# wborgeaud/python-bulletproofs

Measured on AMD Instinct MI355X. Metric: Pippenger MSM scalar-point pairs/sec at n=2^20, higher is better.
Workload: dtype u32x9 (29-bit limbs, 256-bit modular integer); 1 GPU; MSM n=2^20 per GPU over secp256k1, uniform 256-bit scalars (SHA-256), points k_i*G, inputs resident in HBM, 64-byte result to host every step; pairs_per_gpu=1048576, pipeline=2 MSMs in flight (bpmi_msm_dev_enqueue / bpmi_msm_finish)

## Files before the change

### python-bulletproofs_amd/csrc/msm_host.hpp

```cpp
#pragma once

struct MsmGraphKey {
  int lane, slot, glv, small, opt_quad, opt_tail, opt_epl, opt_hist_threads, opt_hist_blocks;
  u32 w0, wcount;
  Segs segs;
  MsmGeom g;
  const void *ws, *pin;
};
struct MsmGraphEntry {
  MsmGraphKey key;
  hipGraph_t graph = nullptr;
  hipGraphExec_t exec = nullptr;
  u32 W = 0, nv = 0, c = 0; int tail = 2; TailOffs to;
};
struct MsmGraphCache { std::vector<MsmGraphEntry> entries; };
static void msm_graphs_clear(bpmi_ctx *ctx) {
  if (!ctx->graphs || ctx->graphs->entries.empty()) return;
  (void)sync_lanes(ctx);
  for (auto &e : ctx->graphs->entries) { if (e.exec) (void)hipGraphExecDestroy(e.exec); if (e.graph) (void)hipGraphDestroy(e.graph); }
  ctx->graphs->entries.clear();
}
static void msm_graph_key(MsmGraphKey &key, const bpmi_ctx *ctx, const MsmPlan &pl, int lane, int slot, const Segs &segs_in, u32 w0, u32 wcount) {
  memset(&key, 0, sizeof(key));
  key.lane = lane; key.slot = slot; key.glv = pl.glv; key.small = pl.small ? 1 : (pl.mid ? 2 : 0); key.opt_quad = ctx->opt_quad; key.opt_tail = ctx->opt_tail; key.opt_epl = ctx->opt_epl;
  key.opt_hist_threads = ctx->opt_hist_threads; key.opt_hist_blocks = ctx->opt_hist_blocks; key.w0 = w0; key.wcount = wcount;
  memcpy(&key.segs, &segs_in, sizeof(Segs)); memcpy(&key.g, &pl.g, sizeof(MsmGeom));
  key.ws = ctx->lane[lane].ws; key.pin = ctx->pend[slot].pin;
}
struct MsmCapture {
  bpmi_ctx *ctx; hipStream_t st; bpmi_ctx::PendingMsm &pd;
  MsmGraphKey key; bool open = false;
  MsmCapture(bpmi_ctx *c, hipStream_t s, bpmi_ctx::PendingMsm &p) : ctx(c), st(s), pd(p) {}
  ~MsmCapture() { if (open) { hipGraph_t g = nullptr; (void)hipStreamEndCapture(st, &g); if (g) (void)hipGraphDestroy(g); (void)hipGetLastError(); } }
  int begin(bool &replayed) {
    replayed = false;
    if (ctx->graphs)
      for (auto &e : ctx->graphs->entries)
        if (!memcmp(&e.key, &key, sizeof(key))) {
          HIPCHK(ctx, hipGraphLaunch(e.exec, st));
          replayed = true;
          return commit(e.W, e.nv, e.c, e.tail, e.to);
        }
    HIPCHK(ctx, hipStreamBeginCapture(st, hipStreamCaptureModeThreadLocal));
    open = true;
    return BPMI_OK;
  }
  int commit(u32 W_, u32 nv_, u32 c_, int tail_, const TailOffs &to_) {
    if (open) {
      MsmGraphEntry e;
      memcpy(&e.key, &key, sizeof(key)); e.W = W_; e.nv = nv_; e.c = c_; e.tail = tail_; e.to = to_;
      open = false;
      HIPCHK(ctx, hipStreamEndCapture(st, &e.graph));
      hipError_t ie = hipGraphInstantiate(&e.exec, e.graph, nullptr, nullptr, 0);
      if (ie != hipSuccess) { (void)hipGraphDestroy(e.graph); return fail(ctx, BPMI_E_HIP, std::string("hipGraphInstantiate: ") + hipGetErrorString(ie)); }
      if (!ctx->graphs) ctx->graphs = new MsmGraphCache();
      if (ctx->graphs->entries.size() >= 48) msm_graphs_clear(ctx);
      ctx->graphs->entries.push_back(e);
      HIPCHK(ctx, hipGraphLaunch(e.exec, st));
    }
    HIPCHK(ctx, hipEventRecord(pd.done, st));
    pd.active = true; pd.W = W_; pd.nv = nv_; pd.c = c_; pd.tail = tail_; pd.to = to_;
    HIPCHK(ctx, hipGetLastError());
    return BPMI_OK;
  }
};

static int msm_queue_mid(bpmi_ctx *ctx, hipStream_t st, const bpmi_ctx::PendingMsm &pd, const Segs &segs, const MsmGeom &g, const MsmWs &w, u32 *E_dst) {
  {
    StageTimer t(ctx, ST_ACCUM, st);
    MidPair mp;
    memset(&mp, 0, sizeof(mp));
    mp.segs[0] = segs; mp.g[0] = g; mp.E[0] = E_dst;
    hipLaunchKernelGGL(k_msm_mid, dim3(g.W, 1, g.nv), dim3(MID_THREADS), 0, st, mp);
  }
  debug_sync(ctx, "k_msm_mid", st);
  if (!ctx->opt_direct) HIPCHK(ctx, hipMemcpyAsync(pd.pin, w.E, 4ull * XYZZ_WORDS * g.W * g.nv, hipMemcpyDeviceToHost, st));
  return BPMI_OK;
}
static int msm_queue_small(bpmi_ctx *ctx, hipStream_t st, const bpmi_ctx::PendingMsm &pd, const Segs &segs, const MsmGeom &g, const MsmWs &w, u32 *E_dst) {
  const uint64_t n = segs.total;
  {
    StageTimer t(ctx, ST_ACCUM, st);
    const u32 threads = (u32)std::min<uint64_t>(256, (n + 63) / 64 * 64);
    const u32 S = (u32)std::min<uint64_t>(64, (n + 255) / 256);
    hipLaunchKernelGGL(k_msm_small, dim3(g.W, S), dim3(threads), 0, st, segs, g, S > 1 ? w.buckets : E_dst);
    if (S > 1) hipLaunchKernelGGL(k_small_combine, dim3(g.W), dim3(64), 0, st, w.buckets, S, E_dst);
  }
  debug_sync(ctx, "k_msm_small", st);
  if (!ctx->opt_direct) HIPCHK(ctx, hipMemcpyAsync(pd.pin, w.E, 4ull * XYZZ_WORDS * g.W, hipMemcpyDeviceToHost, st));
  return BPMI_OK;
}
static void msm_queue_sort_lds(bpmi_ctx *ctx, hipStream_t st, const Segs &segs, const MsmGeom &g, const MsmWs &w, const MsmRecode *rec = nullptr) {
  {
    StageTimer t(ctx, ST_DIGITS, st);
    const u32 ht = ctx->opt_hist_threads > 0 ? (u32)ctx->opt_hist_threads : 1024u;
    const u32 hb = (u32)std::min<uint64_t>(((uint64_t)(rec ? rec->real.n : g.n) + ht - 1) / ht, ctx->opt_hist_blocks > 0 ? (u32)ctx->opt_hist_blocks : 256u);
    CoarseScanOut so = {nullptr, nullptr, nullptr, nullptr};
    if (ctx->opt_histscan && !rec) { so.coarse_off = w.coarse_off; so.coarse_cursor = w.coarse_cursor; so.offG = w.off + g.G; so.ticket = w.coarse_hist + PART_MAX + 2; }
    if (rec) hipLaunchKernelGGL(k_fixed_recode, dim3(hb), dim3(ht), 0, st, rec->sc, rec->real, rec->n_scalars, rec->R, rec->Wv, g, w.P, w.coarse_hist, w.dig16, w.negs);
    else hipLaunchKernelGGL(k_coarse_hist, dim3(hb), dim3(ht), 0, st, segs, g, w.P, w.coarse_hist, w.dig16, w.negs, so);
  }
  debug_sync(ctx, "ST_DIGITS", st);
  if (!ctx->opt_histscan || rec) {
    StageTimer t(ctx, ST_SCAN, st);
    hipLaunchKernelGGL(k_coarse_scan, dim3(1), dim3(1024), 0, st, w.coarse_hist, w.P, w.coarse_off, w.coarse_cursor, w.off + g.G);
  }
  debug_sync(ctx, "ST_SCAN", st);
  {
    StageTimer t(ctx, ST_SCATTER, st);
    const u32 TS = g.n >= (1u << 19) ? PT_MAX : 4096u;
    hipLaunchKernelGGL(k_partition, dim3((g.n + TS - 1) / TS, g.W), dim3(PT_THREADS), 0, st, g, w.P, TS, w.coarse_off, w.coarse_cursor, w.dig16, w.negs, w.dig,
                       w.hist, w.coarse_hist + PART_MAX);
    const u32 nft = (u32)(((size_t)g.n * g.W + FINE_TILE - 1) / FINE_TILE);
    const u32 *any_heavy = w.coarse_hist + PART_MAX;
    if (!g.inblock) hipLaunchKernelGGL(k_fine_hist_heavy, dim3(nft), dim3(256), 0, st, g, w.P, w.coarse_off, w.dig, w.coarse_off + w.P, any_heavy, w.hist);
    hipLaunchKernelGGL(k_fine_sort_part, dim3(w.P), dim3(FINE_THREADS), 0, st, g, w.coarse_off, w.dig, w.hist, w.off, w.cursor, w.chunk_key, w.sidx, w.buckets);
    if (!g.inblock) hipLaunchKernelGGL(k_fine_scatter_heavy, dim3(nft), dim3(256), 0, st, g, w.P, w.coarse_off, w.dig, w.coarse_off + w.P, any_heavy, w.cursor, w.sidx);
    if (g.runs) {
      const u32 cap = msm_runs_cap(*ctx, g), nblk = msm_runs_blocks(g);
      const RunTable rt = {w.run_order, w.run_counts, w.run_flags, msm_runs_bins(cap), cap};
      hipLaunchKernelGGL(k_runs_hist, dim3(nblk), dim3(256), 0, st, g, w.off, rt);
      hipLaunchKernelGGL(k_runs_scatter, dim3(nblk), dim3(256), 0, st, g, w.off, rt);
    }
  }
  debug_sync(ctx, "ST_SCATTER", st);
}
static void msm_queue_sort_atomic(bpmi_ctx *ctx, hipStream_t st, const Segs &segs, const MsmGeom &g, const MsmWs &w) {
  const u32 nblk_n = (u32)std::min<uint64_t>(((uint64_t)g.n + 255) / 256, 8192);
  {
    StageTimer t(ctx, ST_DIGITS, st);
    hipLaunchKernelGGL(k_digits_hist, dim3(nblk_n), dim3(256), 0, st, segs, g, w.dig, w.hist);
  }
  debug_sync(ctx, "ST_DIGITS", st);
  {
    StageTimer t(ctx, ST_SCAN, st);
    hipLaunchKernelGGL(k_scan_partials, dim3(w.nscan_blocks), dim3(256), 0, st, w.hist, g.G, w.bsum);
    hipLaunchKernelGGL(k_scan_top, dim3(1), dim3(1024), 0, st, w.bsum, w.nscan_blocks, w.off, g.G);
    hipLaunchKernelGGL(k_scan_final, dim3(w.nscan_blocks), dim3(256), 0, st, w.hist, g.G, w.bsum, w.off, w.cursor);
  }
  debug_sync(ctx, "ST_SCAN", st);
  {
    StageTimer t(ctx, ST_SCATTER, st);
    hipLaunchKernelGGL(k_scatter, dim3(nblk_n), dim3(256), 0, st, g, w.dig, w.cursor, w.sidx);
    hipLaunchKernelGGL(k_chunk_keys, dim3((g.G + 255) / 256), dim3(256), 0, st, g, w.off, w.chunk_key);
  }
  debug_sync(ctx, "ST_SCATTER", st);
}
static int msm_queue_sort(bpmi_ctx *ctx, hipStream_t st, const Segs &segs, const MsmGeom &g, const MsmWs &w, const MsmRecode *rec = nullptr) {
  {
    StageTimer t(ctx, ST_MISC, st);
    if (w.P) HIPCHK(ctx, hipMemsetAsync(w.coarse_hist, 0, 4ull * COARSE_HIST_WORDS, st));
    else {
      HIPCHK(ctx, hipMemsetAsync(w.hist, 0, 4ull * g.G, st));
      HIPCHK(ctx, hipMemsetAsync(w.buckets, 0, 4ull * XYZZ_WORDS * g.G, st));
    }
  }
  debug_sync(ctx, "ST_MISC", st);
  if (w.P) msm_queue_sort_lds(ctx, st, segs, g, w, rec);
  else msm_queue_sort_atomic(ctx, st, segs, g, w);
  return BPMI_OK;
}
static int msm_queue_accumulate(bpmi_ctx *ctx, const MsmMode &mode, int lane, hipStream_t st, const Segs &segs, const MsmGeom &g, const MsmWs &w, bool glv) {
  const bool own_acc = mode.chained && ctx->opt_accum_stream && ctx->stream_acc;
  hipStream_t st_acc = own_acc ? ctx->stream_acc : st;
  Lane &l = ctx->lane[lane];
  if (own_acc) {
    HIPCHK(ctx, hipEventRecord(l.ev_sorted, st));
    HIPCHK(ctx, hipStreamWaitEvent(st_acc, l.ev_sorted, 0));
  } else if (mode.chained && !mode.free_run && ctx->accum_chain_lane >= 0 && ctx->accum_chain_lane != lane)
    HIPCHK(ctx, hipStreamWaitEvent(st, ctx->lane[ctx->accum_chain_lane].ev_accum, 0));
  {
    StageTimer t(ctx, ST_ACCUM, st_acc);
    auto kern = glv ? (g.fuse ? k_accum_l0<true, true> : k_accum_l0<true, false>) : (g.fuse ? k_accum_l0<false, true> : k_accum_l0<false, false>);
    const u32 *long_run = g.runs ? w.run_flags + RUN_FLAG_WORD : nullptr;
    if (g.runs) {
      auto runs = (!glv && segs_one_dense(segs)) ? k_accum_runs<true> : k_accum_runs<false>;
      hipLaunchKernelGGL(runs, dim3((g.G + 255) / 256), dim3(256), 0, st_acc, segs, g, w.off, w.sidx, w.run_order, w.run_flags, w.buckets);
    }
    hipLaunchKernelGGL(kern, dim3((w.nchunks + 255) / 256), dim3(256), 0, st_acc, segs, g, w.off, w.chunk_key, w.sidx, w.buckets, w.rec_key[0], w.rec_pt[0], long_run);
  }
  if (own_acc) {
    HIPCHK(ctx, hipEventRecord(l.ev_accum, st_acc));
    HIPCHK(ctx, hipStreamWaitEvent(st, l.ev_accum, 0));
  } else if (mode.chained) { HIPCHK(ctx, hipEventRecord(l.ev_accum, st)); ctx->accum_chain_lane = lane; }
  debug_sync(ctx, "ST_ACCUM", st);
  return BPMI_OK;
}
static void msm_queue_segscan(bpmi_ctx *ctx, hipStream_t st, const MsmGeom &g, const MsmWs &w) {
  {
    StageTimer t(ctx, ST_SEGSCAN, st);
    u32 R = w.rec0_max;
    int level = 1, src = 0;
    u32 *ticket = (w.P && ctx->opt_segfuse) ? w.coarse_hist + PART_MAX + 1 : nullptr;
    const u32 *long_run = g.runs ? w.run_flags + RUN_FLAG_WORD : nullptr;
    for (;;) {
      const u32 nb = (R + 255) / 256;
      if (nb > 128u || nb <= 1u) ticket = nullptr;
      hipLaunchKernelGGL(k_segscan, dim3(nb), dim3(256), 0, st, g, w.off, level, w.rec_key[src], w.rec_pt[src],
                         w.rec_key[src ^ 1], w.rec_pt[src ^ 1], w.buckets, ticket, long_run);
      if (g_debug_sync) { fprintf(stderr, "[bpmi] segscan level %d nb %u R %u\n", level, nb, R); debug_sync(ctx, "segscan level", st); }
      if (nb <= 1 || ticket) break;
      R = 2 * nb;
      src ^= 1;
      level++;
    }
  }
  debug_sync(ctx, "ST_SEGSCAN", st);
}
static TailOffs msm_queue_reduce(bpmi_ctx *ctx, hipStream_t st, const MsmGeom &g, const MsmWs &w, u32 *E_red) {
  const MsmReducePlan r = msm_reduce_plan(g, *ctx);
  {
    StageTimer t(ctx, ST_BREDUCE, st);
    if (g.B <= 256u) {
      if (ctx->opt_quad) hipLaunchKernelGGL(k_window_weighted_small_quad, dim3(g.W), dim3(g.B < 16u ? 64u : 4u * g.B), 0, st, g, w.buckets, E_red);
      else hipLaunchKernelGGL(k_window_weighted_small, dim3(g.W), dim3(g.B < 64u ? 64u : g.B), 0, st, g, w.buckets, E_red);
    } else {
      hipLaunchKernelGGL(k_digit_sums, dim3(r.grid1), dim3(256), 0, st, w.buckets, w.D, r.j1);
      if (ctx->opt_quad && ctx->opt_final_spread == 1 && w.P)
        hipLaunchKernelGGL(k_digit_final_spread<0>, dim3(g.W * 64u), dim3(64), 0, st, w.D, w.F, w.coarse_hist + PART_MAX + 8, E_red, r.j2, r.j2top, r.top_w);
      else if (ctx->opt_quad && ctx->opt_final_spread >= 2) {
        if (ctx->opt_final_spread == 2) hipLaunchKernelGGL(k_digit_final_spread<1>, dim3(g.W * 64u), dim3(64), 0, st, w.D, w.F, nullptr, E_red, r.j2, r.j2top, r.top_w);
        else hipLaunchKernelGGL(k_digit_final_spread<1>, dim3(g.W * 16u), dim3(256), 0, st, w.D, w.F, nullptr, E_red, r.j2, r.j2top, r.top_w);
        hipLaunchKernelGGL(k_digit_final_spread<2>, dim3(g.W * 4u), dim3(64), 0, st, w.D, w.F, nullptr, E_red, r.j2, r.j2top, r.top_w);
      }
      else if (ctx->opt_quad) hipLaunchKernelGGL(k_digit_final_quad, dim3(g.W * 4u), dim3(1024), 0, st, w.D, E_red, r.j2, r.j2top, r.top_w);
      else hipLaunchKernelGGL(k_digit_final, dim3(g.W * 4u), dim3(256), 0, st, w.D, E_red, r.j2, r.j2top, r.top_w);
    }
  }
  debug_sync(ctx, "ST_BREDUCE", st);
  return r.to;
}
static int msm_queue_tail(bpmi_ctx *ctx, hipStream_t st, const bpmi_ctx::PendingMsm &pd, const MsmGeom &g, const MsmWs &w, int tail, const TailOffs &to) {
  StageTimer t(ctx, ST_TAIL, st);
  if (tail == 1) {
    hipLaunchKernelGGL(k_tail, dim3(1), dim3(64), 0, st, w.E, g.W, g.c, to, ctx->opt_direct ? (u32 *)pd.pin : w.out);
    if (!ctx->opt_direct) HIPCHK(ctx, hipMemcpyAsync(pd.pin, w.out, 64, hipMemcpyDeviceToHost, st));
  } else if (!ctx->opt_direct)
    HIPCHK(ctx, hipMemcpyAsync(pd.pin, w.E, 4ull * XYZZ_WORDS * g.W * g.nv, hipMemcpyDeviceToHost, st));
  return BPMI_OK;
}

static int msm_enqueue(bpmi_ctx *ctx, const MsmMode &mode, int lane, int slot, const Segs &segs_in, u32 w0 = 0, u32 wcount = 0, int phase = 0,
                       const MsmRecode *rec = nullptr) {
  Segs segs = segs_in;
  const uint64_t n = segs.total;
  bpmi_ctx::PendingMsm &pd = ctx->pend[slot];
  if (pd.active) return fail(ctx, BPMI_E_STATE, "an MSM is still pending in this slot (bpmi_msm_finish it first)");
  if (n == 0) return BPMI_OK;
  if (n > BPMI_MAX_N) return fail(ctx, BPMI_E_ARG, "n exceeds BPMI_MAX_N");
  const MsmPlan pl = rec ? rec->plan : msm_pick_geometry(*ctx, mode, n, w0, wcount);
  MsmGeom g = pl.g;
  MsmWs w;
  msm_layout(g, w, nullptr, pl.glv);
  int rc = ensure_lane(ctx, lane);
  if (rc) return rc;
  rc = ensure_ws(ctx, w.total, lane);
  if (rc) return rc;
  msm_layout(g, w, (char *)ctx->lane[lane].ws, pl.glv);
  hipStream_t st = ctx->lane[lane].stream;
  rc = ensure_pin_slot(ctx, slot, std::max<size_t>(4096, 4ull * XYZZ_WORDS * g.W * 4));
  if (rc) return rc;
  const bool sort_ahead = !pl.mid && !pl.small && !pl.glv;
  if (phase == 1) {
    if (!sort_ahead) return BPMI_OK;
    if ((rc = msm_queue_sort(ctx, st, segs, g, w))) return rc;
    HIPCHK(ctx, hipGetLastError());
    return BPMI_OK;
  }
  MsmCapture cap(ctx, st, pd);
  if (phase == 0 && ctx->opt_graph && !ctx->prof && !g_debug_sync && !mode.chained && !rec) {
    msm_graph_key(cap.key, ctx, pl, lane, slot, segs_in, w0, wcount);
    bool replayed;
    rc = cap.begin(replayed);
    if (rc || replayed) return rc;
  }
  u32 *const E_dst = ctx->opt_direct ? (u32 *)pd.pin : w.E;
  if (pl.glv) {
    StageTimer t(ctx, ST_DIGITS, st);
    hipLaunchKernelGGL(k_glv_prepare, dim3((u32)((n + 255) / 256)), dim3(256), 0, st, segs, (u32)n, w.glv_sub, w.glv_neg, w.glv_bx);
    segs.glv_sub = w.glv_sub; segs.glv_neg = w.glv_neg; segs.glv_bx = w.glv_bx;
  }
  TailOffs to;
  memset(&to, 0, sizeof(to));
  to.nv = 1;
  int tail = 2;
  if (pl.mid) {
    g.nv = to.nv = mid_parts(*ctx, n);
    if ((rc = msm_queue_mid(ctx, st, pd, segs, g, w, E_dst))) return rc;
  } else if (pl.small) {
    if ((rc = msm_queue_small(ctx, st, pd, segs, g, w, E_dst))) return rc;
  } else {
    ctx->lane[lane].run_planned = g.runs; ctx->lane[lane].run_flags = w.P ? w.run_flags : nullptr;
    if (!(phase == 2 && sort_ahead) && (rc = msm_queue_sort(ctx, st, segs, g, w, rec))) return rc;
    if ((rc = msm_queue_accumulate(ctx, mode, lane, st, segs, g, w, pl.glv))) return rc;
    msm_queue_segscan(ctx, st, g, w);
    tail = wcount ? 2 : (ctx->opt_tail ? ctx->opt_tail : 2);
    to = msm_queue_reduce(ctx, st, g, w, tail == 1 ? w.E : E_dst);
    if ((rc = msm_queue_tail(ctx, st, pd, g, w, tail, to))) return rc;
  }
  return cap.commit(g.W, g.nv, g.c, tail, to);
}
static void msm_abandon_pending(bpmi_ctx *ctx, unsigned mine) {
  (void)sync_lanes(ctx);
  for (int s = 0; s < BPMI_LANES; s++) if ((mine >> s) & 1u) ctx->pend[s].active = false;
}
static int msm_finish(bpmi_ctx *ctx, int slot, uint8_t out[64]) {
  bpmi_ctx::PendingMsm &pd = ctx->pend[slot];
  if (!pd.active) { memset(out, 0, 64); return BPMI_OK; }
  pd.active = false;
  HIPCHK(ctx, wait_event(ctx, pd.done));
  const void *pin = pd.pin;
  if (pd.tail == 1) {
    memcpy(out, pin, 64);
  } else {
    bpmi_host::tail_combine(out, (const u32 *)pin, pd.W, pd.c, pd.to);
  }
  return BPMI_OK;
}
static int msm_run_split(bpmi_ctx *ctx, const Segs &segs, uint8_t out[64]) {
  const u32 c = pick_window_bits(*ctx, segs.total), W = 255u / c + 1u, Wa = W / 2;
  int rc = ensure_lane(ctx, 1);
  if (rc) return rc;
  HIPCHK(ctx, hipEventRecord(ctx->ev_fork, ctx->stream));
  HIPCHK(ctx, hipStreamWaitEvent(ctx->lane[1].stream, ctx->ev_fork, 0));
  rc = msm_enqueue(ctx, MsmMode{}, 0, 0, segs, 0, Wa);
  if (rc) return rc;
  rc = msm_enqueue(ctx, MsmMode{}, 1, 1, segs, Wa, W - Wa);
  if (rc) { msm_abandon_pending(ctx, 1u); return rc; }
  bpmi_ctx::PendingMsm &p0 = ctx->pend[0], &p1 = ctx->pend[1];
  HIPCHK(ctx, hipStreamSynchronize(ctx->stream));
  HIPCHK(ctx, hipStreamSynchronize(ctx->lane[1].stream));
  const size_t b0 = 4ull * XYZZ_WORDS * p0.W * p0.nv, b1 = 4ull * XYZZ_WORDS * p1.W * p1.nv;
  std::vector<u32> E((b0 + b1) / 4);
  memcpy(E.data(), p0.pin, b0);
  memcpy((char *)E.data() + b0, p1.pin, b1);
  bpmi_host::tail_combine(out, E.data(), W, c, p0.to);
  p0.active = p1.active = false;
  return BPMI_OK;
}
static int msm_finish_pair(bpmi_ctx *ctx, uint8_t out0[64], uint8_t out1[64]);
static int msm_run_sliced(bpmi_ctx *ctx, const Segs &segs, uint64_t K, uint8_t out[64]) {
  for (int s = 0; s < 2; s++) if (ctx->pend[s].active || ctx->pend[s].async) return fail(ctx, BPMI_E_STATE, "an MSM is still pending in this slot (bpmi_msm_finish it first)");
  int rc = ensure_lane(ctx, 1);
  if (rc) return rc;
  HIPCHK(ctx, hipEventRecord(ctx->ev_fork, ctx->stream));
  HIPCHK(ctx, hipStreamWaitEvent(ctx->lane[1].stream, ctx->ev_fork, 0));
  const uint64_t total = segs.total, per = (total + K - 1) / K;
  bpmi_host::pt acc;
  bpmi_host::pt_set_inf(acc);
  unsigned mine = 0;
  MsmMode mode;
  mode.chained = per >= (1u << 19);
  auto leave = [&](int code) { ctx->accum_chain_lane = -1; if (code) msm_abandon_pending(ctx, mine); return code; };
  auto take = [&](int slot) -> int {
    uint8_t part[64];
    mine &= ~(1u << slot);
    const int r = msm_finish(ctx, slot, part);
    if (r) return r;
    bpmi_host::pt p;
    bpmi_host::pt_from_affine(p, part);
    bpmi_host::pt_add(acc, acc, p);
    return BPMI_OK;
  };
  ctx->accum_chain_lane = -1;
  for (uint64_t k = 0; k < K; k++) {
    const int lane = (int)(k & 1);
    if (k >= 2) { rc = take(lane); if (rc) return leave(rc); }
    const MsmSlice sl = msm_slice(total, per, k);
    rc = msm_enqueue(ctx, mode, lane, lane, segs_slice(segs, sl.lo, sl.cnt));
    if (rc) return leave(rc);
    mine |= 1u << lane;
  }
  {
    uint8_t part[2][64];
    mine = 0;
    rc = msm_finish_pair(ctx, part[0], part[1]);
    if (rc) return leave(rc);
    for (uint64_t k = K - 2; k < K; k++) {
      bpmi_host::pt p;
      bpmi_host::pt_from_affine(p, part[k & 1]);
      bpmi_host::pt_add(acc, acc, p);
    }
  }
  bpmi_host::pt_to_affine(out, acc);
  return leave(BPMI_OK);
}
static int msm_run(bpmi_ctx *ctx, const Segs &segs, uint8_t out[64]) {
  if (segs.total > BPMI_MAX_N) return fail(ctx, BPMI_E_ARG, "n exceeds BPMI_MAX_N");
  {
    const uint64_t K = msm_slice_count(*ctx, segs);
    if (K > 1) return msm_run_sliced(ctx, segs, K, out);
  }
  if (ctx->opt_split == 1 && segs.total >= 2) return msm_run_split(ctx, segs, out);
  int rc = msm_enqueue(ctx, MsmMode{}, 0, 0, segs);
  if (rc) return rc;
  return msm_finish(ctx, 0, out);
}
static int msm_finish_pair(bpmi_ctx *ctx, uint8_t out0[64], uint8_t out1[64]) {
  if (!ctx->opt_tail_thread || !ctx->pend[0].active || !ctx->pend[1].active) {
    const int rc = msm_finish(ctx, 0, out0), rc1 = msm_finish(ctx, 1, out1);
    return rc ? rc : rc1;
  }
  if (!ctx->helper) ctx->helper = new HostHelper();
  bpmi_ctx::PendingMsm &pd = ctx->pend[1];
  hipError_t e1 = hipSuccess;
  const int dev = ctx->device;
  ctx->helper->submit([&pd, &e1, out1, dev, ctx] {
    (void)hipSetDevice(dev);
    e1 = wait_event(ctx, pd.done);
    if (e1 != hipSuccess) return;
    if (pd.tail == 1) memcpy(out1, pd.pin, 64);
    else bpmi_host::tail_combine(out1, (const u32 *)pd.pin, pd.W, pd.c, pd.to);
  });
  const int rc = msm_finish(ctx, 0, out0);
  ctx->helper->wait();
  pd.active = false;
  if (rc) return rc;
  HIPCHK(ctx, e1);
  return BPMI_OK;
}
static int msm_enqueue_small_pair(bpmi_ctx *ctx, const Segs &s0, const Segs &s1, bool mid) {
  bpmi_ctx::PendingMsm &p0 = ctx->pend[0], &p1 = ctx->pend[1];
  if (p0.active || p1.active) return fail(ctx, BPMI_E_STATE, "an MSM is still pending in this slot (bpmi_msm_finish it first)");
  SmallPair sp;
  CombinePair cp;
  MidPair mp;
  memset(&mp, 0, sizeof(mp));
  const Segs *ss[2] = {&s0, &s1};
  size_t off[2], total = 0;
  MsmWs w[2];
  MsmGeom gg[2];
  const u32 c = mid ? MID_C : SMALL_C;
  for (int j = 0; j < 2; j++) {
    MsmGeom &g = gg[j];
    memset(&g, 0, sizeof(g));
    g.n = ss[j]->total; g.c = c; g.W = 255u / g.c + 1u; g.w0 = 0; g.B = 1u << (g.c - 1); g.G = g.W * g.B; g.L = 8; g.nv = 1;
    msm_layout(g, w[j], nullptr);
    off[j] = total;
    total += align_up(w[j].total, 256);
  }
  int rc = ensure_ws(ctx, total);
  if (rc) return rc;
  const u32 parts = mid ? mid_parts(*ctx, std::max(s0.total, s1.total)) : 1u;
  const size_t eb = 4ull * XYZZ_WORDS * gg[0].W * parts;
  for (int j = 0; j < 2; j++) { rc = ensure_pin_slot(ctx, j, eb); if (rc) return rc; }
  u32 Smax = 1, threads = 64;
  for (int j = 0; j < 2; j++) {
    msm_layout(gg[j], w[j], (char *)ctx->lane[0].ws + off[j]);
    const uint64_t n = ss[j]->total;
    const u32 S = (u32)std::min<uint64_t>(64, (n + 255) / 256);
    u32 *const E_dst = ctx->opt_direct ? (u32 *)ctx->pend[j].pin : w[j].E;
    sp.segs[j] = *ss[j]; sp.g[j] = gg[j]; sp.S[j] = S; sp.out[j] = S > 1 ? w[j].buckets : E_dst;
    cp.part[j] = w[j].buckets; cp.S[j] = S; cp.E[j] = E_dst;
    mp.segs[j] = *ss[j]; mp.g[j] = gg[j]; mp.E[j] = E_dst;
    Smax = std::max(Smax, S);
    threads = std::max(threads, (u32)std::min<uint64_t>(256, (n + 63) / 64 * 64));
  }
  hipStream_t st = ctx->stream;
  {
    StageTimer t(ctx, ST_ACCUM, st);
    if (mid) hipLaunchKernelGGL(k_msm_mid, dim3(gg[0].W, 2, parts), dim3(MID_THREADS), 0, st, mp);
    else {
      hipLaunchKernelGGL(k_msm_small_pair, dim3(gg[0].W, Smax, 2), dim3(threads), 0, st, sp);
      if (Smax > 1) hipLaunchKernelGGL(k_small_combine_pair, dim3(gg[0].W, 2), dim3(64), 0, st, cp);
    }
  }
  debug_sync(ctx, "k_msm_small_pair / k_msm_mid", st);
  TailOffs to;
  memset(&to, 0, sizeof(to));
  to.nv = parts;
  unsigned mine = 0;
  auto queue_results = [&]() -> int {
    for (int j = 0; j < 2; j++) {
      bpmi_ctx::PendingMsm &pd = ctx->pend[j];
      if (!ctx->opt_direct) HIPCHK(ctx, hipMemcpyAsync(pd.pin, w[j].E, eb, hipMemcpyDeviceToHost, st));
      HIPCHK(ctx, hipEventRecord(pd.done, st));
      pd.active = true; pd.W = gg[j].W; pd.nv = parts; pd.c = c; pd.tail = 2; pd.to = to;
      mine |= 1u << j;
    }
    HIPCHK(ctx, hipGetLastError());
    return BPMI_OK;
  };
  rc = queue_results();
  if (rc && mine) msm_abandon_pending(ctx, mine);
  return rc;
}
static int msm_run_pair(bpmi_ctx *ctx, const Segs &s0, uint8_t out0[64], const Segs &s1, uint8_t out1[64]) {
  if (s0.total > BPMI_MAX_N || s1.total > BPMI_MAX_N) return fail(ctx, BPMI_E_ARG, "n exceeds BPMI_MAX_N");
  {
    const uint64_t small_max = ctx->opt_small < 0 ? 0 : (ctx->opt_small ? (uint64_t)ctx->opt_small : SMALL_N_DEFAULT);
    const uint64_t mid_min = ctx->opt_mid_min > 0 ? (uint64_t)ctx->opt_mid_min : MID_MIN_DEFAULT;
    const uint64_t big = std::max<uint64_t>(s0.total, s1.total);
    const bool mid = ctx->opt_mid_min >= 0 && big >= mid_min && big <= MID_NMAX && ctx->opt_glv <= 0;
    if (ctx->opt_pair1 && ctx->opt_c == 0 && s0.total && s1.total && (mid || big <= small_max)) {
      int rc = msm_enqueue_small_pair(ctx, s0, s1, mid);
      if (rc) return rc;
      return msm_finish_pair(ctx, out0, out1);
    }
  }
  int rc = ensure_lane(ctx, 1);
  if (rc) return rc;
  HIPCHK(ctx, hipEventRecord(ctx->ev_fork, ctx->stream));
  HIPCHK(ctx, hipStreamWaitEvent(ctx->lane[1].stream, ctx->ev_fork, 0));
  const bool big = s0.total >= (1u << 19) && s1.total >= (1u << 19);
  const bool sched = ctx->opt_pair_sched && big && !ctx->opt_graph;
  const bool chain = sched || (ctx->opt_pair_chain && big);
  MsmMode mode;
  mode.chained = chain;
  mode.beside = ctx->opt_pair_rounds != 1 && big;
  if (chain) ctx->accum_chain_lane = -1;
  auto leave = [&](int code) { if (chain) ctx->accum_chain_lane = -1; return code; };
  const bool phases = sched || (ctx->opt_pair_phases && !chain && !ctx->opt_graph && s0.total >= (1u << 15) && s1.total >= (1u << 15));
  if (phases) {
    rc = msm_enqueue(ctx, mode, 0, 0, s0, 0, 0, 1);
    if (rc == BPMI_OK) rc = msm_enqueue(ctx, mode, 1, 1, s1, 0, 0, 1);
    if (rc) { msm_abandon_pending(ctx, 0u); return leave(rc); }
    if (sched) {
      hipError_t e = hipEventRecord(ctx->ev_join, ctx->lane[1].stream);
      if (e == hipSuccess) e = hipStreamWaitEvent(ctx->stream, ctx->ev_join, 0);
      if (e != hipSuccess) { msm_abandon_pending(ctx, 0u); return leave(fail(ctx, BPMI_E_HIP, std::string("msm_run_pair: ") + hipGetErrorString(e))); }
    }
  }
  rc = msm_enqueue(ctx, mode, 0, 0, s0, 0, 0, phases ? 2 : 0);
  if (rc == BPMI_OK) {
    rc = msm_enqueue(ctx, mode, 1, 1, s1, 0, 0, phases ? 2 : 0);
    if (rc) msm_abandon_pending(ctx, 1u);
  }
  leave(0);
  if (rc) return rc;
  return msm_finish_pair(ctx, out0, out1);
}
```

### python-bulletproofs_amd/csrc/msm_kernels.hpp

```cpp
#pragma once

__device__ __forceinline__ void raise_priority(u32 on) { if (on) __builtin_amdgcn_s_setprio(3); }
__device__ __forceinline__ u32 geom_wide(const MsmGeom &g, u32 w) { return (g.top2 && w + g.top2 >= g.W) ? 1u : 0u; }
__device__ __forceinline__ u32 geom_slot(const MsmGeom &g, u32 w) { return (g.top2 && w + g.top2 > g.W) ? 2u * w + g.top2 - g.W : w; }

__device__ __forceinline__ bool load_digit_source(sc &s, const Segs &segs, u32 i) {
  if (segs.glv_sub) {
    const uint4 t = *reinterpret_cast<const uint4 *>(segs.glv_sub + 4ull * i);
    s.v[0] = t.x; s.v[1] = t.y; s.v[2] = t.z; s.v[3] = t.w;
    s.v[4] = s.v[5] = s.v[6] = s.v[7] = 0;
    return segs.glv_neg[i] != 0;
  }
  load_words8(s.v, seg_scalar(segs, i));
  sc_reduce_once(s);
  const bool neg = sc_is_high(s);
  if (neg) sc_neg(s, s);
  return neg;
}
template <typename F>
__device__ __forceinline__ bool for_each_digit_raw(const Segs &segs, const MsmGeom &g, u32 i, F f) {
  sc s;
  const bool neg = load_digit_source(s, segs, i);
  u32 carry = 0;
  const u32 wend = g.w0 + g.W;
  for (u32 w = 0; w < wend; w++) {
    const u32 wd = g.c + geom_wide(g, w);
    const u32 t = (s.v[0] & ((1u << wd) - 1u)) + carry;
#pragma unroll
    for (int k = 0; k < 7; k++) s.v[k] = (u32)((((u64)s.v[k + 1] << 32) | s.v[k]) >> wd);
    s.v[7] >>= wd;
    u32 b, sign;
    if (t > (1u << (wd - 1u))) { b = (1u << wd) - t; sign = 1; carry = 1; }
    else { b = t; sign = 0; carry = 0; }
    if (w >= g.w0) f(w - g.w0, b, b ? sign : 0u);
  }
  return neg;
}
template <typename F>
__device__ __forceinline__ void for_each_digit(const Segs &segs, const MsmGeom &g, u32 i, F f) {
  sc s;
  const bool neg = load_digit_source(s, segs, i);
  u32 carry = 0;
  const u32 wend = g.w0 + g.W;
  for (u32 w = 0; w < wend; w++) {
    const u32 wd = g.c + geom_wide(g, w);
    const u32 t = (s.v[0] & ((1u << wd) - 1u)) + carry;
#pragma unroll
    for (int k = 0; k < 7; k++) s.v[k] = (u32)((((u64)s.v[k + 1] << 32) | s.v[k]) >> wd);
    s.v[7] >>= wd;
    u32 b, sign;
    if (t > (1u << (wd - 1u))) { b = (1u << wd) - t; sign = 1; carry = 1; }
    else { b = t; sign = 0; carry = 0; }
    if (w >= g.w0) f(w - g.w0, b, b ? (sign ^ (u32)neg) : 0u);
  }
}

__global__ void __launch_bounds__(256) k_glv_prepare(Segs segs, u32 n, u32 *__restrict__ sub, unsigned char *__restrict__ neg, u32 *__restrict__ bx) {
  const u32 i = blockIdx.x * blockDim.x + threadIdx.x;
  if (i >= n) return;
  sc k;
  load_words8(k.v, seg_scalar(segs, i));
  sc_reduce_once(k);
  u32 k1[4], k2[4];
  bool n1, n2;
  glv_split(k1, n1, k2, n2, k);
  uint4 *o = reinterpret_cast<uint4 *>(sub + 8ull * i);
  o[0] = make_uint4(k1[0], k1[1], k1[2], k1[3]);
  o[1] = make_uint4(k2[0], k2[1], k2[2], k2[3]);
  neg[2ull * i] = n1 ? 1 : 0;
  neg[2ull * i + 1] = n2 ? 1 : 0;
  u32 w[8];
  load_words8(w, seg_point(segs, i));
  fe x, r, c;
  fe_from_words(x, w);
  fe_mul_beta(r, x);
  fe_canon(c, r);
  fe_to_words(w, c);
  store_words8(bx + 8ull * i, w);
}

__global__ void __launch_bounds__(256) k_digits_hist(Segs segs, MsmGeom g, u32 *__restrict__ dig, u32 *__restrict__ hist) {
  raise_priority(g.prio & PRIO_SORT);
  const u32 stride = gridDim.x * blockDim.x;
  for (u32 i = blockIdx.x * blockDim.x + threadIdx.x; i < g.n; i += stride) {
    for_each_digit(segs, g, i, [&](u32 w, u32 b, u32 sign) {
      dig[(u64)w * g.n + i] = b | (sign << 31);
      const u32 key = b ? (w * g.B + b - 1u) : 0xFFFFFFFFu;
      const unsigned long long act = __ballot(1);
      const u32 first = __builtin_amdgcn_readfirstlane(key);
      const unsigned long long same = __ballot(key == first);
      if (same == act) {
        if (first != 0xFFFFFFFFu) {
          const u32 lane_rank = __builtin_amdgcn_mbcnt_hi((u32)(act >> 32), __builtin_amdgcn_mbcnt_lo((u32)act, 0));
          if (lane_rank == 0) atomicAdd(&hist[first], (u32)__popcll(act));
        }
      } else if (b) {
        atomicAdd(&hist[key], 1u);
      }
    });
  }
}

#define FINE_CAP 12288
#define DIG_NONE 0xFFFFu
struct CoarseScanOut { u32 *coarse_off, *coarse_cursor, *offG, *ticket; };
__global__ void __launch_bounds__(1024) k_coarse_hist(Segs segs, MsmGeom g, u32 P, u32 *coarse_hist, unsigned short *__restrict__ dig16,
                                                     unsigned char *__restrict__ negs, CoarseScanOut scan) {
  raise_priority(g.prio & PRIO_SORT);
  __shared__ u32 lh[PART_MAX];
  __shared__ u32 s_last;
  for (u32 p = threadIdx.x; p < P; p += blockDim.x) lh[p] = 0;
  __syncthreads();
  const u32 Bc = g.B >> 8;
  const u32 stride = gridDim.x * blockDim.x;
  for (u32 i = blockIdx.x * blockDim.x + threadIdx.x; i < g.n; i += stride) {
    const bool neg = for_each_digit_raw(segs, g, i, [&](u32 w, u32 b, u32 dsign) {
      dig16[(u64)w * g.n + i] = (unsigned short)(b ? ((b - 1u) | (dsign << 15)) : DIG_NONE);
      if (b) atomicAdd(&lh[geom_slot(g, w) * Bc + ((b - 1u) >> 8)], 1u);
    });
    negs[i] = neg ? 1 : 0;
  }
  __syncthreads();
  for (u32 p = threadIdx.x; p < P; p += blockDim.x) { const u32 v = lh[p]; if (v) atomicAdd(&coarse_hist[p], v); }
  if (!scan.ticket) return;
  __threadfence();
  __syncthreads();
  if (threadIdx.x == 0) s_last = (atomicAdd(scan.ticket, 1u) == gridDim.x - 1u) ? 1u : 0u;
  __syncthreads();
  if (!s_last) return;
  __threadfence();
  const u32 tid = threadIdx.x, nt = blockDim.x, per = (P + nt - 1u) / nt;
  u32 loc[8], sum = 0;
#pragma unroll
  for (u32 k = 0; k < 8u; k++) {
    const u32 idx = tid * per + k;
    loc[k] = (k < per && idx < P) ? __atomic_load_n(&coarse_hist[idx], __ATOMIC_RELAXED) : 0u;
    sum += loc[k];
  }
  lh[tid] = sum;
  __syncthreads();
  for (u32 d = 1; d < nt; d <<= 1) {
    const u32 v = tid >= d ? lh[tid - d] : 0u;
    __syncthreads();
    lh[tid] += v;
    __syncthreads();
  }
  u32 excl = lh[tid] - sum;
#pragma unroll
  for (u32 k = 0; k < 8u; k++) {
    const u32 idx = tid * per + k;
    if (k < per && idx < P) { scan.coarse_off[idx] = excl; scan.coarse_cursor[idx] = excl; excl += loc[k]; }
  }
  if (tid == nt - 1u) { scan.coarse_off[P] = lh[tid]; *scan.offG = lh[tid]; }
}
__global__ void __launch_bounds__(1024) k_coarse_scan(const u32 *__restrict__ coarse_hist, u32 P, u32 *__restrict__ coarse_off,
                                                      u32 *__restrict__ coarse_cursor, u32 *__restrict__ offG) {
  __shared__ u32 sh[1024];
  const u32 tid = threadIdx.x;
  const u32 a = (2u * tid < P) ? coarse_hist[2u * tid] : 0u, b = (2u * tid + 1u < P) ? coarse_hist[2u * tid + 1u] : 0u;
  sh[tid] = a + b;
  __syncthreads();
  for (u32 d = 1; d < 1024u; d <<= 1) {
    const u32 v = tid >= d ? sh[tid - d] : 0u;
    __syncthreads();
    sh[tid] += v;
    __syncthreads();
  }
  const u32 excl = sh[tid] - (a + b);
  if (2u * tid < P) { coarse_off[2u * tid] = excl; coarse_cursor[2u * tid] = excl; }
  if (2u * tid + 1u < P) { coarse_off[2u * tid + 1u] = excl + a; coarse_cursor[2u * tid + 1u] = excl + a; }
  if (tid == 1023u) { coarse_off[P] = sh[1023]; *offG = sh[1023]; }
}
#define PT_MAX 16384
#define PT_THREADS 1024u
struct alignas(8) PartSigns { unsigned char b[8]; };
__global__ void __launch_bounds__(PT_THREADS) k_partition(MsmGeom g, u32 P, u32 TS, const u32 *__restrict__ coarse_off, u32 *__restrict__ coarse_cursor,
                                                          const unsigned short *__restrict__ dig16, const unsigned char *__restrict__ negs,
                                                          u32 *__restrict__ part, u32 *__restrict__ fine_hist, u32 *__restrict__ any_heavy) {
  constexpr u32 THREADS = PT_THREADS;
  static_assert((PT_MAX / 8u) % THREADS == 0u, "k_partition: whole vectors per thread");
  constexpr u32 NV = PT_MAX / 8u / THREADS;
  raise_priority(g.prio & PRIO_SORT);
  __shared__ u32 cnt[128], excl[128], delta[128];
  __shared__ u32 s_out[PT_MAX];
  const u32 w = blockIdx.y, tid = threadIdx.x;
  const u32 Bc0 = g.B >> 8, Bc = Bc0 << geom_wide(g, w), pbase = geom_slot(g, w) * Bc0;
  const u32 lin = blockIdx.y * gridDim.x + blockIdx.x, nblk = gridDim.x * gridDim.y;
  if (!g.inblock) for (u32 p = lin; p < P; p += nblk) {
    if (coarse_off[p + 1] - coarse_off[p] > FINE_CAP) {
      if (tid < 256u) fine_hist[p * 256u + tid] = 0;
      if (tid == 0) *any_heavy = 1u;
    }
  }
  const u32 i0 = blockIdx.x * TS;
  const u32 i1 = (i0 + TS < g.n) ? i0 + TS : g.n;
  const u64 wn = (u64)w * g.n;
  const unsigned short *dw = dig16 + wn;
  const u32 span = i1 - i0, mis = (u32)((0u - (u32)((wn + i0) & 7ull)) & 7u);
  const u32 head = mis < span ? mis : span;
  const u32 a0 = i0 + head, nvec = (i1 - a0) >> 3, t0 = a0 + 8u * nvec;
  const u32 nscal = head + (i1 - t0);
  const u32 is = tid < head ? i0 + tid : t0 + (tid - head);
  uint4 cv[NV];
  PartSigns sv[NV];
  u32 cs = DIG_NONE, ss = 0;
#pragma unroll
  for (u32 k = 0; k < NV; k++) {
    const u32 v = k * THREADS + tid;
    cv[k] = make_uint4(0xFFFFFFFFu, 0xFFFFFFFFu, 0xFFFFFFFFu, 0xFFFFFFFFu);
    if (v < nvec) {
      cv[k] = *reinterpret_cast<const uint4 *>(dw + a0 + 8u * v);
      __builtin_memcpy(&sv[k], negs + a0 + 8u * v, 8);
    }
  }
  if (tid < nscal) { cs = dw[is]; ss = negs[is]; }
  if (tid < 128u) cnt[tid] = 0;
  __syncthreads();
#pragma unroll
  for (u32 k = 0; k < NV; k++) {
    const u32 q[4] = {cv[k].x, cv[k].y, cv[k].z, cv[k].w};
#pragma unroll
    for (u32 e = 0; e < 8u; e++) {
      const u32 code = (q[e >> 1] >> (16u * (e & 1u))) & 0xFFFFu;
      if (code != DIG_NONE) atomicAdd(&cnt[(code & 0x7FFFu) >> 8], 1u);
    }
  }
  if (cs != DIG_NONE) atomicAdd(&cnt[(cs & 0x7FFFu) >> 8], 1u);
  __syncthreads();
  u32 c = 0;
  if (tid < 128u) { c = tid < Bc ? cnt[tid] : 0u; excl[tid] = c; }
  __syncthreads();
  for (u32 d = 1; d < 128u; d <<= 1) {
    u32 v = 0;
    if (tid < 128u && tid >= d) v = excl[tid - d];
    __syncthreads();
    if (tid < 128u) excl[tid] += v;
    __syncthreads();
  }
  if (tid < 128u) {
    const u32 start = excl[tid] - c;
    excl[tid] = start;
    cnt[tid] = start;
    if (c) delta[tid] = atomicAdd(&coarse_cursor[pbase + tid], c) - start;
  }
  __syncthreads();
#pragma unroll
  for (u32 k = 0; k < NV; k++) {
    const u32 q[4] = {cv[k].x, cv[k].y, cv[k].z, cv[k].w};
    const u32 ib = a0 + 8u * (k * THREADS + tid);
#pragma unroll
    for (u32 e = 0; e < 8u; e++) {
      const u32 code = (q[e >> 1] >> (16u * (e & 1u))) & 0xFFFFu;
      if (code != DIG_NONE) {
        const u32 kk = code & 0x7FFFu;
        s_out[atomicAdd(&cnt[kk >> 8], 1u)] = ((kk & 255u) << 24) | (((code >> 15) ^ (u32)sv[k].b[e]) << 23) | (ib + e);
      }
    }
  }
  if (cs != DIG_NONE) {
    const u32 kk = cs & 0x7FFFu;
    s_out[atomicAdd(&cnt[kk >> 8], 1u)] = ((kk & 255u) << 24) | (((cs >> 15) ^ ss) << 23) | is;
  }
  __syncthreads();
  const u32 wave = tid >> 6, lane = tid & 63u, nwaves = THREADS >> 6;
  for (u32 p = wave; p < Bc; p += nwaves) {
    const u32 lo = excl[p], hi = cnt[p], dl = delta[p];
    for (u32 j = lo + lane; j < hi; j += 64u) part[dl + j] = s_out[j];
  }
}
#define CHUNK_FILL_OWN 16u
__device__ __forceinline__ void fill_chunk_keys(u32 *__restrict__ chunk_key, u32 L, u32 key, u32 lo, u32 hi) {
  const u32 t0 = (lo + L - 1u) / L;
  const u32 t1 = hi > lo ? (u32)(((u64)hi + L - 1u) / L) : t0;
  const bool big = t1 - t0 > CHUNK_FILL_OWN;
  if (!big) for (u32 t = t0; t < t1; t++) chunk_key[t] = key;
  unsigned long long m = __ballot(big);
  const u32 lane = __builtin_amdgcn_mbcnt_hi(~0u, __builtin_amdgcn_mbcnt_lo(~0u, 0u));
  while (m) {
    const int src = __ffsll((long long)m) - 1;
    m &= m - 1ull;
    const u32 k = (u32)__shfl((int)key, src, 64), a = (u32)__shfl((int)t0, src, 64), b = (u32)__shfl((int)t1, src, 64);
    for (u32 t = a + lane; t < b; t += 64u) chunk_key[t] = k;
  }
}
#define FINE_THREADS 512
__device__ __forceinline__ u32 lds_take_slot(u32 *bins, u32 bin) {
  const u32 lane = __builtin_amdgcn_mbcnt_hi(~0u, __builtin_amdgcn_mbcnt_lo(~0u, 0u));
  u32 pos = 0;
  bool done = false;
  for (int it = 0; it < 4; it++) {
    const unsigned long long rem = __ballot(!done);
    if (rem == 0ull) break;
    const u32 first = (u32)__shfl((int)bin, __ffsll((long long)rem) - 1, 64);
    const bool match = !done && bin == first;
    const unsigned long long m = __ballot(match);
    if (match) {
      const u32 rank = (u32)__popcll(m & ((1ull << lane) - 1ull));
      u32 basepos = 0;
      if (rank == 0) basepos = atomicAdd(&bins[first], (u32)__popcll(m));
      basepos = (u32)__shfl((int)basepos, __ffsll((long long)m) - 1, 64);
      pos = basepos + rank;
      done = true;
    }
  }
  if (!done) pos = atomicAdd(&bins[bin], 1u);
  return pos;
}
__global__ void __launch_bounds__(FINE_THREADS) k_fine_sort_part(MsmGeom g, const u32 *__restrict__ coarse_off, const u32 *__restrict__ part,
                                                                  const u32 *__restrict__ fine_hist, u32 *__restrict__ off, u32 *__restrict__ cursor,
                                                                  u32 *__restrict__ chunk_key, u32 *__restrict__ sidx, u32 *__restrict__ buckets) {
  raise_priority(g.prio & PRIO_SORT);
  __shared__ u32 bins[256];
  __shared__ u32 s_out[FINE_CAP];
  const u32 p = blockIdx.x, tid = threadIdx.x;
  const u32 base = coarse_off[p], m = coarse_off[p + 1] - base;
  const bool big = m > FINE_CAP;
  const bool heavy = big && !g.inblock;
  if (tid < 256u) bins[tid] = heavy ? fine_hist[p * 256u + tid] : 0u;
  __syncthreads();
  if (!heavy) {
    if (big) for (u32 i = tid; i < m; i += FINE_THREADS) (void)lds_take_slot(bins, part[base + i] >> 24);
    else for (u32 i = tid; i < m; i += FINE_THREADS) atomicAdd(&bins[part[base + i] >> 24], 1u);
    __syncthreads();
  }
  u32 cnt = 0;
  if (tid < 256u) cnt = bins[tid];
  for (u32 d = 1; d < 256u; d <<= 1) {
    u32 v = 0;
    if (tid < 256u && tid >= d) v = bins[tid - d];
    __syncthreads();
    if (tid < 256u) bins[tid] += v;
    __syncthreads();
  }
  if (tid < 256u) {
    const u32 start = bins[tid] - cnt;
    const u32 key = p * 256u + tid;
    off[key] = base + start;
    fill_chunk_keys(chunk_key, g.L, key, base + start, base + start + cnt);
    if (heavy) cursor[key] = base + start;
    if (cnt == 0) {
      xyzz inf;
      xyzz_set_inf(inf);
      xyzz_store_g(buckets + (u64)key * XYZZ_WORDS, inf);
    }
  }
  if (heavy) return;
  __syncthreads();
  if (tid < 256u) bins[tid] -= cnt;
  __syncthreads();
  if (big) {
    for (u32 i = tid; i < m; i += FINE_THREADS) {
      const u32 e = part[base + i];
      sidx[base + lds_take_slot(bins, e >> 24)] = (e & 0x7FFFFFu) | ((e & 0x800000u) << 8);
    }
    return;
  }
  for (u32 i = tid; i < m; i += FINE_THREADS) {
    const u32 e = part[base + i];
    s_out[atomicAdd(&bins[e >> 24], 1u)] = (e & 0x7FFFFFu) | ((e & 0x800000u) << 8);
  }
  __syncthreads();
  for (u32 i = tid; i < m; i += FINE_THREADS) sidx[base + i] = s_out[i];
}
#define FINE_BINS 4096
struct FineTile {
  u32 j0, j1;
  u32 p_first;
};
__device__ __forceinline__ FineTile fine_tile_setup(const u32 *__restrict__ coarse_off, u32 P, u32 E, u32 *s_off) {
  for (u32 i = threadIdx.x; i <= P; i += 256u) s_off[i] = coarse_off[i];
  __syncthreads();
  FineTile t;
  t.j0 = blockIdx.x * FINE_TILE;
  t.j1 = (t.j0 + FINE_TILE < E) ? t.j0 + FINE_TILE : E;
  u32 lo = 0, hi = P;
  while (hi - lo > 1) { const u32 mid = (lo + hi) >> 1; if (s_off[mid] <= t.j0) lo = mid; else hi = mid; }
  t.p_first = lo;
  return t;
}
__device__ __forceinline__ u32 fine_partition_of(const u32 *s_off, u32 P, u32 pcur, u32 j) {
  u32 lo = pcur + 1u, hi = P - 1u;
  while (lo < hi) { const u32 mid = (lo + hi) >> 1; if (s_off[mid + 1] > j) hi = mid; else lo = mid + 1u; }
  return lo;
}
__global__ void __launch_bounds__(256) k_fine_hist_heavy(MsmGeom g, u32 P, const u32 *__restrict__ coarse_off, const u32 *__restrict__ part,
                                                         const u32 *__restrict__ offE, const u32 *__restrict__ any_heavy, u32 *__restrict__ fine_hist) {
  raise_priority(g.prio & PRIO_SORT);
  __shared__ u32 s_off[PART_MAX + 1];
  __shared__ u32 bins[FINE_BINS];
  if (!*any_heavy) return;
  const u32 E = offE[0];
  if (blockIdx.x * FINE_TILE >= E) return;
  const FineTile t = fine_tile_setup(coarse_off, P, E, s_off);
  for (u32 i = threadIdx.x; i < FINE_BINS; i += 256u) bins[i] = 0;
  __syncthreads();
  const u32 g_first = t.p_first * 256u;
  u32 pcur = t.p_first, bound = s_off[pcur + 1];
  bool heavy = bound - s_off[pcur] > FINE_CAP;
  for (u32 j = t.j0 + threadIdx.x; j < t.j1; j += 256u) {
    if (j >= bound) { pcur = fine_partition_of(s_off, P, pcur, j); bound = s_off[pcur + 1]; heavy = bound - s_off[pcur] > FINE_CAP; }
    if (heavy) {
      const u32 key = pcur * 256u + (part[j] >> 24);
      const u32 rel = key - g_first;
      if (rel < FINE_BINS) atomicAdd(&bins[rel], 1u); else atomicAdd(&fine_hist[key], 1u);
    }
  }
  __syncthreads();
  for (u32 i = threadIdx.x; i < FINE_BINS; i += 256u) { const u32 v = bins[i]; if (v) atomicAdd(&fine_hist[g_first + i], v); }
}
__global__ void __launch_bounds__(256) k_fine_scatter_heavy(MsmGeom g, u32 P, const u32 *__restrict__ coarse_off, const u32 *__restrict__ part,
                                                            const u32 *__restrict__ offE, const u32 *__restrict__ any_heavy, u32 *__restrict__ cursor,
                                                            u32 *__restrict__ sidx) {
  raise_priority(g.prio & PRIO_SORT);
  __shared__ u32 s_off[PART_MAX + 1];
  __shared__ u32 bins[FINE_BINS];
  if (!*any_heavy) return;
  const u32 E = offE[0];
  if (blockIdx.x * FINE_TILE >= E) return;
  const FineTile t = fine_tile_setup(coarse_off, P, E, s_off);
  for (u32 i = threadIdx.x; i < FINE_BINS; i += 256u) bins[i] = 0;
  __syncthreads();
  const u32 g_first = t.p_first * 256u;
  u32 pcur = t.p_first, bound = s_off[pcur + 1];
  bool heavy = bound - s_off[pcur] > FINE_CAP;
  for (u32 j = t.j0 + threadIdx.x; j < t.j1; j += 256u) {
    if (j >= bound) { pcur = fine_partition_of(s_off, P, pcur, j); bound = s_off[pcur + 1]; heavy = bound - s_off[pcur] > FINE_CAP; }
    if (heavy) {
      const u32 rel = pcur * 256u + (part[j] >> 24) - g_first;
      if (rel < FINE_BINS) atomicAdd(&bins[rel], 1u);
    }
  }
  __syncthreads();
  for (u32 i = threadIdx.x; i < FINE_BINS; i += 256u) { const u32 v = bins[i]; if (v) bins[i] = atomicAdd(&cursor[g_first + i], v); }
  __syncthreads();
  pcur = t.p_first; bound = s_off[pcur + 1];
  heavy = bound - s_off[pcur] > FINE_CAP;
  for (u32 j = t.j0 + threadIdx.x; j < t.j1; j += 256u) {
    if (j >= bound) { pcur = fine_partition_of(s_off, P, pcur, j); bound = s_off[pcur + 1]; heavy = bound - s_off[pcur] > FINE_CAP; }
    if (heavy) {
      const u32 e = part[j];
      const u32 key = pcur * 256u + (e >> 24);
      const u32 rel = key - g_first;
      const u32 pos = (rel < FINE_BINS) ? atomicAdd(&bins[rel], 1u) : atomicAdd(&cursor[key], 1u);
      sidx[pos] = (e & 0x7FFFFFu) | ((e & 0x800000u) << 8);
    }
  }
}
__global__ void __launch_bounds__(256) k_chunk_keys(MsmGeom g, const u32 *__restrict__ off, u32 *__restrict__ chunk_key) {
  raise_priority(g.prio & PRIO_SORT);
  const u32 key = blockIdx.x * blockDim.x + threadIdx.x;
  const bool valid = key < g.G;
  const u32 lo = valid ? off[key] : 0u, hi = valid ? off[key + 1] : 0u;
  fill_chunk_keys(chunk_key, g.L, key, lo, hi);
}

__global__ void __launch_bounds__(256) k_scan_partials(const u32 *__restrict__ hist, u32 G, u32 *__restrict__ bsum) {
  __shared__ u32 red[256];
  const u32 base = blockIdx.x * SCAN_TILE + threadIdx.x * SCAN_PER_THREAD;
  u32 s = 0;
#pragma unroll
  for (int k = 0; k < SCAN_PER_THREAD; k++) { const u32 j = base + k; if (j < G) s += hist[j]; }
  red[threadIdx.x] = s;
  __syncthreads();
  for (int d = 128; d > 0; d >>= 1) { if (threadIdx.x < d) red[threadIdx.x] += red[threadIdx.x + d]; __syncthreads(); }
  if (threadIdx.x == 0) bsum[blockIdx.x] = red[0];
}
__global__ void __launch_bounds__(1024) k_scan_top(u32 *__restrict__ bsum, u32 nb, u32 *__restrict__ off, u32 G) {
  __shared__ u32 sh[1024];
  u32 running = 0;
  for (u32 base = 0; base < nb; base += 1024) {
    const u32 j = base + threadIdx.x;
    const u32 v = j < nb ? bsum[j] : 0;
    sh[threadIdx.x] = v;
    __syncthreads();
    for (int d = 1; d < 1024; d <<= 1) {
      u32 t = threadIdx.x >= d ? sh[threadIdx.x - d] : 0;
      __syncthreads();
      sh[threadIdx.x] += t;
      __syncthreads();
    }
    if (j < nb) bsum[j] = running + sh[threadIdx.x] - v;
    const u32 tot = sh[1023];
    __syncthreads();
    running += tot;
  }
  if (threadIdx.x == 0) off[G] = running;
}
__global__ void __launch_bounds__(256) k_scan_final(const u32 *__restrict__ hist, u32 G, const u32 *__restrict__ bsum,
                                                    u32 *__restrict__ off, u32 *__restrict__ cursor) {
  __shared__ u32 sh[256];
  const u32 base = blockIdx.x * SCAN_TILE + threadIdx.x * SCAN_PER_THREAD;
  u32 v[SCAN_PER_THREAD];
  u32 s = 0;
#pragma unroll
  for (int k = 0; k < SCAN_PER_THREAD; k++) { const u32 j = base + k; v[k] = j < G ? hist[j] : 0; s += v[k]; }
  sh[threadIdx.x] = s;
  __syncthreads();
  for (int d = 1; d < 256; d <<= 1) {
    u32 t = threadIdx.x >= d ? sh[threadIdx.x - d] : 0;
    __syncthreads();
    sh[threadIdx.x] += t;
    __syncthreads();
  }
  u32 run = bsum[blockIdx.x] + sh[threadIdx.x] - s;
#pragma unroll
  for (int k = 0; k < SCAN_PER_THREAD; k++) {
    const u32 j = base + k;
    if (j < G) { off[j] = run; cursor[j] = run; }
    run += v[k];
  }
}

__global__ void __launch_bounds__(256) k_scatter(MsmGeom g, const u32 *__restrict__ dig, u32 *__restrict__ cursor,
                                                 u32 *__restrict__ sidx) {
  raise_priority(g.prio & PRIO_SORT);
  const u32 stride = gridDim.x * blockDim.x;
  for (u32 w = 0; w < g.W; w++) {
    for (u32 i = blockIdx.x * blockDim.x + threadIdx.x; i < g.n; i += stride) {
      const u32 d = dig[(u64)w * g.n + i];
      const u32 b = d & 0x7FFFFFFFu;
      const u32 key = b ? (w * g.B + b - 1u) : 0xFFFFFFFFu;
      const unsigned long long act = __ballot(1);
      const u32 first = __builtin_amdgcn_readfirstlane(key);
      const unsigned long long same = __ballot(key == first);
      u32 pos = 0;
      if (same == act) {
        if (first != 0xFFFFFFFFu) {
          const u32 lane_rank = __builtin_amdgcn_mbcnt_hi((u32)(act >> 32), __builtin_amdgcn_mbcnt_lo((u32)act, 0));
          u32 basepos = 0;
          if (lane_rank == 0) basepos = atomicAdd(&cursor[first], (u32)__popcll(act));
          basepos = __builtin_amdgcn_readfirstlane(basepos);
          pos = basepos + lane_rank;
        }
      } else if (b) {
        pos = atomicAdd(&cursor[key], 1u);
      }
      if (b) sidx[pos] = i | (d & 0x80000000u);
    }
  }
}

__device__ __forceinline__ void xyzz_shfl_up(xyzz &r, const xyzz &a, int d) {
#pragma unroll
  for (int i = 0; i < 9; i++) {
    r.X.v[i] = (u32)__shfl_up((int)a.X.v[i], d, 64);
    r.Y.v[i] = (u32)__shfl_up((int)a.Y.v[i], d, 64);
    r.ZZ.v[i] = (u32)__shfl_up((int)a.ZZ.v[i], d, 64);
    r.ZZZ.v[i] = (u32)__shfl_up((int)a.ZZZ.v[i], d, 64);
  }
}
template <bool GLV, bool FUSE> __global__ void __launch_bounds__(256) k_accum_l0(Segs segs, MsmGeom g, const u32 *__restrict__ off,
                                                  const u32 *__restrict__ chunk_key, const u32 *__restrict__ sidx,
                                                  u32 *__restrict__ buckets, u32 *__restrict__ rec_key, u32 *__restrict__ rec_pt,
                                                  const u32 *__restrict__ long_run) {
  __shared__ u32 s_head[FUSE ? 256 * LDS_STRIDE : 1];
  if (long_run && !*long_run) return;
  const u32 E = off[g.G];
  const u64 t = (u64)blockIdx.x * blockDim.x + threadIdx.x;
  const u64 start = t * g.L;
  const bool valid = start < E;
  if (!FUSE) { if (!valid) return; }
  else if (__ballot(valid) == 0ull) return;
  const u32 end = (u32)((start + g.L < E) ? start + g.L : E);
  xyzz acc;
  xyzz_set_inf(acc);
  u32 cur = valid ? chunk_key[t] : 0u;
  const u32 hk = cur;
  bool first = true;
  if (valid) {
  u32 boundary = off[cur + 1];
  u32 boundary2 = off[cur + 2 < g.G ? cur + 2 : g.G];
  u32 e_next = sidx[start];
  u32 e_next2 = (start + 1 < end) ? sidx[start + 1] : 0u;
  u32 w_next[16];
  load_entry_point<GLV>(w_next, segs, e_next & 0x7FFFFFFFu);
  for (u32 j = (u32)start; j < end; j++) {
    const u32 e = e_next;
    affine P;
    affine_from_words(P, w_next);
    asm volatile("" : "+v"(P.x.v[0]), "+v"(P.x.v[1]), "+v"(P.x.v[2]), "+v"(P.x.v[3]), "+v"(P.x.v[4]), "+v"(P.x.v[5]), "+v"(P.x.v[6]),
                 "+v"(P.x.v[7]), "+v"(P.x.v[8]), "+v"(P.y.v[0]), "+v"(P.y.v[1]), "+v"(P.y.v[2]), "+v"(P.y.v[3]), "+v"(P.y.v[4]),
                 "+v"(P.y.v[5]), "+v"(P.y.v[6]), "+v"(P.y.v[7]), "+v"(P.y.v[8]));
    if (j + 1 < end) {
      e_next = e_next2;
      if (j + 2 < end) e_next2 = sidx[j + 2];
      load_entry_point<GLV>(w_next, segs, e_next & 0x7FFFFFFFu);
    }
    if (j == boundary) {
      if (first) {
        if (FUSE) xyzz_store(s_head + threadIdx.x * LDS_STRIDE, acc);
        else { rec_key[2 * t] = cur; xyzz_store_g(rec_pt + (2 * t) * XYZZ_WORDS, acc); }
        first = false;
      }
      else xyzz_store_g(buckets + (u64)cur * XYZZ_WORDS, acc);
      xyzz_set_inf(acc);
      cur++; boundary = boundary2;
      if (boundary == j) {
        u32 steps = 0;
        do { cur++; boundary = off[cur + 1]; steps++; } while (boundary == j && steps < 8u);
        if (boundary == j) {
          u32 lo = cur + 1u, hi = g.G - 1u;
          while (lo < hi) { const u32 mid = (lo + hi) >> 1; if (off[mid + 1] > j) hi = mid; else lo = mid + 1u; }
          cur = lo; boundary = off[cur + 1];
        }
      }
      boundary2 = off[cur + 2 < g.G ? cur + 2 : g.G];
    }
    xyzz_madd_signed(acc, P, (e >> 31) != 0);
  }
  }
  if (!FUSE) {
    if (first) {
      rec_key[2 * t] = cur; xyzz_store_g(rec_pt + (2 * t) * XYZZ_WORDS, acc);
      xyzz_set_inf(acc);
    }
    rec_key[2 * t + 1] = cur;
    xyzz_store_g(rec_pt + (2 * t + 1) * XYZZ_WORDS, acc);
    return;
  }
  const u32 lane = threadIdx.x & 63u;
  const u32 gw = (u32)(t >> 6);
  const bool single = first;
  const u32 tk = cur;
  const u32 prev_tk = (u32)__shfl_up((int)tk, 1, 64);
  const bool link = valid && lane > 0u && prev_tk == hk;
  bool F = !(valid && single && link);
  for (u32 d = 1; d < 64u; d <<= 1) {
    const bool take = !F;
    if (__ballot(take) == 0ull) break;
    xyzz o;
    xyzz_shfl_up(o, acc, (int)d);
    const bool oF = __shfl_up((int)F, (int)d, 64) != 0;
    if (take) { xyzz_add(acc, o, acc); F = oF; }
  }
  const u32 first_key = (u32)__shfl((int)hk, 0, 64);
  const bool next_valid = __shfl_down((int)valid, 1, 64) != 0, next_link = __shfl_down((int)link, 1, 64) != 0;
  const bool last = valid && (lane == 63u || !next_valid);
  xyzz Sp;
  xyzz_shfl_up(Sp, acc, 1);
  const bool s_done = valid && (last || !next_link);
  const bool s_is_head = tk == first_key;
  {
    u32 *dst = s_is_head ? rec_pt + (u64)(2u * gw) * XYZZ_WORDS : (last ? rec_pt + (u64)(2u * gw + 1u) * XYZZ_WORDS : buckets + (u64)tk * XYZZ_WORDS);
    if (s_done) xyzz_store_g(dst, acc);
  }
  if (last) {
    rec_key[2u * gw + 1u] = tk;
    if (s_is_head) {
      xyzz_set_inf(acc);
      xyzz_store_g(rec_pt + (u64)(2u * gw + 1u) * XYZZ_WORDS, acc);
    }
  }
  const bool has_head = valid && !single;
  if (__ballot(has_head) != 0ull) {
    if (has_head) xyzz_load(acc, s_head + threadIdx.x * LDS_STRIDE); else xyzz_set_inf(acc);
    if (__ballot(has_head && link) != 0ull) { if (has_head && link) xyzz_add(acc, Sp, acc); }
    u32 *dst = (hk == first_key) ? rec_pt + (u64)(2u * gw) * XYZZ_WORDS : buckets + (u64)hk * XYZZ_WORDS;
    if (has_head) xyzz_store_g(dst, acc);
  }
  if (lane == 0u) rec_key[2u * gw] = first_key;
}

__device__ __forceinline__ u32 records_at_level(u32 E, u32 L, u32 fuse, int level, bool &is_final) {
  is_final = false;
  if (E == 0) return 0;
  const u32 chunks = (E + L - 1) / L;
  u32 R = 2u * (fuse ? (chunks + 63u) / 64u : chunks);
  for (int l = 1; l < level; l++) {
    const u32 nb = (R + 255u) / 256u;
    if (nb <= 1) return 0;
    R = 2u * nb;
  }
  is_final = ((R + 255u) / 256u) <= 1;
  return R;
}

__global__ void __launch_bounds__(256) k_segscan(MsmGeom g, const u32 *__restrict__ off, int level,
                                                 const u32 *in_key, const u32 *in_pt,
                                                 u32 *out_key, u32 *out_pt, u32 *__restrict__ buckets, u32 *ticket, const u32 *__restrict__ long_run) {
  if (long_run && !*long_run) return;
  raise_priority(g.prio & PRIO_SCAN);
  __shared__ u32 s_key[256];
  __shared__ u32 s_val[256 * LDS_STRIDE];
  __shared__ u32 s_last;
  bool is_final;
  u32 R = records_at_level(off[g.G], g.L, g.fuse, level, is_final);
  u32 nb = (R + 255u) / 256u;
  if (blockIdx.x >= nb) return;
  const u32 tid = threadIdx.x;
  u32 blk = blockIdx.x;
  for (;;) {
    const u32 j = blk * 256u + tid;
    const bool valid = j < R;
    const u32 key = valid ? in_key[j] : 0xFFFFFFFFu;
    xyzz val;
    if (valid) xyzz_load_g(val, in_pt + (u64)j * XYZZ_WORDS); else xyzz_set_inf(val);
    s_key[tid] = key;
    __syncthreads();
    for (u32 d = 1; d < 256; d <<= 1) {
      const bool act = valid && tid >= d && s_key[tid - d] == key;
      if (!__syncthreads_or(act)) break;
      xyzz_store(s_val + tid * LDS_STRIDE, val);
      __syncthreads();
      if (act) {
        xyzz other;
        xyzz_load(other, s_val + (tid - d) * LDS_STRIDE);
        xyzz_add(val, other, val);
      }
      __syncthreads();
    }
    const u32 last_idx = (R - blk * 256u >= 256u) ? 255u : (R - blk * 256u - 1u);
    const bool run_end = valid && ((tid == last_idx) || (s_key[tid + (tid < 255u ? 1u : 0u)] != key));
    if (run_end) {
      const u32 first_key = s_key[0], last_key = s_key[last_idx];
      const bool to_bucket = is_final || (key != first_key && key != last_key);
      const bool is_head = !to_bucket && (key == first_key);
      const u32 slot = 2u * blk + (is_head ? 0u : 1u);
      u32 *dst = to_bucket ? buckets + (u64)key * XYZZ_WORDS : out_pt + (u64)slot * XYZZ_WORDS;
      if (!to_bucket) out_key[slot] = key;
      xyzz_store_g(dst, val);
      if (is_head && first_key == last_key) {
        xyzz inf;
        xyzz_set_inf(inf);
        out_key[slot + 1u] = key;
        xyzz_store_g(out_pt + (u64)(slot + 1u) * XYZZ_WORDS, inf);
      }
    }
    if (is_final || !ticket || nb > 128u) return;
    __threadfence();
    __syncthreads();
    if (tid == 0) s_last = (atomicAdd(ticket, 1u) == nb - 1u) ? 1u : 0u;
    __syncthreads();
    if (!s_last) return;
    __threadfence();
    R = 2u * nb; nb = 1; blk = 0; is_final = true;
    in_key = out_key; in_pt = out_pt;
  }
}

struct RunTable { u32 *order, *counts, *flags; u32 nbins, cap; };
template <u32 N> __device__ __forceinline__ void run_lengths(u32 (&len)[N], const u32 *__restrict__ off, u32 k0, u32 stride, u32 k1) {
#pragma unroll
  for (u32 k = 0; k < N; k++) { const u32 key = k0 + k * stride; len[k] = key < k1 ? off[key + 1] - off[key] : 0u; }
}
__global__ void __launch_bounds__(256) k_runs_hist(MsmGeom g, const u32 *__restrict__ off, RunTable rt) {
  raise_priority(g.prio & PRIO_SORT);
  __shared__ u32 bins[RUN_BINS];
  for (u32 i = threadIdx.x; i < rt.nbins; i += 256u) bins[i] = 0;
  __syncthreads();
  const u32 k0 = blockIdx.x * RUN_SLICE, k1 = (k0 + RUN_SLICE < g.G) ? k0 + RUN_SLICE : g.G;
  u32 len[RUN_SLICE / 256u];
  run_lengths(len, off, k0 + threadIdx.x, 256u, k1);
  bool longer = false;
#pragma unroll
  for (u32 k = 0; k < RUN_SLICE / 256u; k++) {
    if (len[k]) atomicAdd(&bins[len[k] < rt.nbins ? len[k] : rt.nbins - 1u], 1u);
    longer |= len[k] > rt.cap;
  }
  __syncthreads();
  for (u32 i = threadIdx.x; i < rt.nbins; i += 256u) rt.counts[(rt.nbins - 1u - i) * gridDim.x + blockIdx.x] = bins[i];
  if (longer) rt.flags[RUN_FLAG_WORD] = 1u;
}
__global__ void __launch_bounds__(256) k_runs_scatter(MsmGeom g, const u32 *__restrict__ off, RunTable rt) {
  raise_priority(g.prio & PRIO_SORT);
  __shared__ u32 s_base[RUN_BINS];
  __shared__ u32 s_wave[4][RUN_BINS];
  __shared__ u32 s_scan[256];
  if (rt.flags[RUN_FLAG_WORD]) return;
  const u32 tid = threadIdx.x, nblk = gridDim.x;
  const u32 wave = tid >> 6, lane = tid & 63u;
  const u32 k0 = blockIdx.x * RUN_SLICE + wave * (RUN_SLICE / 4u);
  const u32 k1 = (k0 + RUN_SLICE / 4u < g.G) ? k0 + RUN_SLICE / 4u : g.G;
  u32 len[RUN_SLICE / 256u];
  run_lengths(len, off, k0 + lane, 64u, k1);
  const u32 M = rt.nbins * nblk, per = ((M + 255u) / 256u + 3u) & ~3u;
  const u32 i0 = tid * per < M ? tid * per : M, i1 = i0 + per < M ? i0 + per : M;
  u32 sum = 0;
  {
    u32 i = i0;
#pragma unroll 4
    for (; i + 4u <= i1; i += 4u) { const uint4 v = *reinterpret_cast<const uint4 *>(rt.counts + i); sum += v.x + v.y + v.z + v.w; }
    for (; i < i1; i++) sum += rt.counts[i];
  }
  s_scan[tid] = sum;
  for (u32 i = tid; i < 4u * RUN_BINS; i += 256u) (&s_wave[0][0])[i] = 0;
  __syncthreads();
  for (u32 d = 1; d < 256u; d <<= 1) {
    const u32 v = tid >= d ? s_scan[tid - d] : 0u;
    __syncthreads();
    s_scan[tid] += v;
    __syncthreads();
  }
  {
    u32 run = s_scan[tid] - sum, row = i0 / nblk, blk = i0 % nblk;
    for (u32 i = i0; i < i1; i++) {
      if (blk == blockIdx.x) s_base[rt.nbins - 1u - row] = run;
      run += rt.counts[i];
      if (++blk == nblk) { blk = 0; row++; }
    }
  }
  if (blockIdx.x == 0 && tid == 255u) rt.flags[RUN_COUNT_WORD] = s_scan[255];
#pragma unroll
  for (u32 k = 0; k < RUN_SLICE / 256u; k++)
    if (len[k]) atomicAdd(&s_wave[wave][len[k] < rt.nbins ? len[k] : rt.nbins - 1u], 1u);
  __syncthreads();
  for (u32 cls = tid; cls < rt.nbins; cls += 256u) {
    u32 b = s_base[cls];
    for (u32 w = 0; w < 4u; w++) { const u32 c = s_wave[w][cls]; s_wave[w][cls] = b; b += c; }
  }
  __syncthreads();
#pragma unroll
  for (u32 k = 0; k < RUN_SLICE / 256u; k++)
    if (len[k]) rt.order[atomicAdd(&s_wave[wave][len[k] < rt.nbins ? len[k] : rt.nbins - 1u], 1u)] = k0 + lane + k * 64u;
}
template <bool DENSE> __device__ __forceinline__ void runs_load_point(u32 w[16], const Segs &segs, u32 idx) {
  if (DENSE) load_words16(w, segs.pts[0] + 16ull * idx);
  else load_entry_point<false>(w, segs, idx);
}
template <bool DENSE> __device__ __forceinline__ void runs_next_entry(affine &P, u32 &e, u32 (&w_next)[16], u32 &e_next, u32 &e_next2, const Segs &segs,
                                                                      const u32 *__restrict__ sidx, u32 j, u32 end) {
  e = e_next;
  affine_from_words(P, w_next);
  asm volatile("" : "+v"(P.x.v[0]), "+v"(P.x.v[1]), "+v"(P.x.v[2]), "+v"(P.x.v[3]), "+v"(P.x.v[4]), "+v"(P.x.v[5]), "+v"(P.x.v[6]),
               "+v"(P.x.v[7]), "+v"(P.x.v[8]), "+v"(P.y.v[0]), "+v"(P.y.v[1]), "+v"(P.y.v[2]), "+v"(P.y.v[3]), "+v"(P.y.v[4]),
               "+v"(P.y.v[5]), "+v"(P.y.v[6]), "+v"(P.y.v[7]), "+v"(P.y.v[8]));
  if (j + 1 < end) {
    e_next = e_next2;
    if (j + 2 < end) e_next2 = sidx[j + 2];
    runs_load_point<DENSE>(w_next, segs, e_next & 0x7FFFFFFFu);
  }
}
__device__ __forceinline__ void runs_signed_y(fe &sy, const fe &y, bool negate) {
  fe_neg(sy, y);
#pragma unroll
  for (int k = 0; k < 9; k++) sy.v[k] = negate ? sy.v[k] : y.v[k];
}
template <bool DENSE> __global__ void __launch_bounds__(256) k_accum_runs(Segs segs, MsmGeom g, const u32 *__restrict__ off, const u32 *__restrict__ sidx,
                                                    const u32 *__restrict__ order, const u32 *__restrict__ flags, u32 *__restrict__ buckets) {
  if (flags[RUN_FLAG_WORD]) return;
  const u32 t = blockIdx.x * blockDim.x + threadIdx.x;
  if (t >= flags[RUN_COUNT_WORD]) return;
  const u32 b = order[t];
  const u32 start = off[b], end = off[b + 1];
  xyzz acc;
  u32 e_next = sidx[start];
  u32 e_next2 = (start + 1 < end) ? sidx[start + 1] : 0u;
  u32 w_next[16];
  runs_load_point<DENSE>(w_next, segs, e_next & 0x7FFFFFFFu);
  u32 j = start, e;
  affine P;
  fe sy;
  runs_next_entry<DENSE>(P, e, w_next, e_next, e_next2, segs, sidx, j, end);
  bool fin = !affine_is_inf(P);
  runs_signed_y(sy, P.y, (e >> 31) != 0);
  if (fin) { acc.X = P.x; fe_carry(acc.Y, sy); fe_set_one(acc.ZZ); fe_set_one(acc.ZZZ); }
  else xyzz_set_inf(acc);
  j++;
  if (j < end) {
    runs_next_entry<DENSE>(P, e, w_next, e_next, e_next2, segs, sidx, j, end);
    if (!affine_is_inf(P)) {
      runs_signed_y(sy, P.y, (e >> 31) != 0);
      if (fin) xyzz_mmadd(acc, acc.X, acc.Y, P.x, sy);
      else { acc.X = P.x; fe_carry(acc.Y, sy); fe_set_one(acc.ZZ); fe_set_one(acc.ZZZ); }
    }
    j++;
  }
  for (; j < end; j++) {
    runs_next_entry<DENSE>(P, e, w_next, e_next, e_next2, segs, sidx, j, end);
    xyzz_madd_signed(acc, P, (e >> 31) != 0);
  }
  xyzz_store_g(buckets + (u64)b * XYZZ_WORDS, acc);
}

__device__ __forceinline__ void block_tree_sum(xyzz &val, u32 *s_val) {
  const u32 tid = threadIdx.x;
  for (u32 d = blockDim.x >> 1; d > 0; d >>= 1) {
    xyzz_store(s_val + tid * LDS_STRIDE, val);
    __syncthreads();
    if (tid < d) {
      xyzz other;
      xyzz_load(other, s_val + (tid + d) * LDS_STRIDE);
      xyzz_add(val, val, other);
    }
    __syncthreads();
  }
}


__device__ __forceinline__ void xyzz_shfl_xor(xyzz &r, const xyzz &a, int mask) {
#pragma unroll
  for (int i = 0; i < 9; i++) {
    r.X.v[i] = (u32)__shfl_xor((int)a.X.v[i], mask, 64);
    r.Y.v[i] = (u32)__shfl_xor((int)a.Y.v[i], mask, 64);
    r.ZZ.v[i] = (u32)__shfl_xor((int)a.ZZ.v[i], mask, 64);
    r.ZZZ.v[i] = (u32)__shfl_xor((int)a.ZZZ.v[i], mask, 64);
  }
}
__device__ __forceinline__ void xyzz_shfl_down(xyzz &r, const xyzz &a, int d) {
#pragma unroll
  for (int i = 0; i < 9; i++) {
    r.X.v[i] = (u32)__shfl_down((int)a.X.v[i], d, 64);
    r.Y.v[i] = (u32)__shfl_down((int)a.Y.v[i], d, 64);
    r.ZZ.v[i] = (u32)__shfl_down((int)a.ZZ.v[i], d, 64);
    r.ZZZ.v[i] = (u32)__shfl_down((int)a.ZZZ.v[i], d, 64);
  }
}
__device__ __forceinline__ void xyzz_shfl_down16(xyzz &r, const xyzz &a, int d) {
#pragma unroll
  for (int i = 0; i < 9; i++) {
    r.X.v[i] = (u32)__shfl_down((int)a.X.v[i], d, 16);
    r.Y.v[i] = (u32)__shfl_down((int)a.Y.v[i], d, 16);
    r.ZZ.v[i] = (u32)__shfl_down((int)a.ZZ.v[i], d, 16);
    r.ZZZ.v[i] = (u32)__shfl_down((int)a.ZZZ.v[i], d, 16);
  }
}

__global__ void __launch_bounds__(256) k_digit_sums(const u32 *__restrict__ X, u32 *__restrict__ D, DigitJobs jobs) {
  raise_priority(jobs.prio);
  u32 ji = 0;
  for (u32 k = 1; k < jobs.njobs; k++) if (blockIdx.x >= jobs.j[k].blk0) ji = k;
  const DigitJob J = jobs.j[ji];
  const u32 t = (blockIdx.x - J.blk0) * blockDim.x + threadIdx.x;
  const u32 GL = J.glanes, lane = t & 63u;
  const u32 grp = lane / GL, l = lane - grp * GL;
  const u32 sum_id = (t >> 6) * J.gpw + grp;
  const bool active = grp < J.gpw && sum_id < J.cnt * J.nsums;
  const u32 a = sum_id / J.nsums, idx = sum_id % J.nsums + 1u;
  xyzz acc;
  xyzz_set_inf(acc);
  const u32 *base = X + ((u64)a * J.in_stride + J.in_off) * XYZZ_WORDS;
  if (active) {
    if (J.type == 0) {
      for (u32 hi = l; ((hi << J.s) | idx) <= J.N; hi += GL) {
        xyzz x;
        xyzz_load_g(x, base + (u64)(((hi << J.s) | idx) - 1u) * XYZZ_WORDS);
        xyzz_add(acc, acc, x);
      }
    } else {
      for (u32 lo = l; lo < (1u << J.s) && ((idx << J.s) | lo) <= J.N; lo += GL) {
        xyzz x;
        xyzz_load_g(x, base + (u64)(((idx << J.s) | lo) - 1u) * XYZZ_WORDS);
        xyzz_add(acc, acc, x);
      }
    }
  }
  if ((GL & (GL - 1u)) == 0u) {
    for (u32 m = 1; m < GL; m <<= 1) {
      xyzz other;
      xyzz_shfl_xor(other, acc, (int)m);
      xyzz_add(acc, acc, other);
    }
  } else {
    u32 d = 1;
    while ((d << 1) < GL) d <<= 1;
    for (u32 width = GL; d > 0 && width > 1; width = d, d >>= 1) {
      xyzz other;
      xyzz_shfl_down(other, acc, (int)d);
      if (!(l < d && l + d < width)) xyzz_set_inf(other);
      xyzz_add(acc, acc, other);
    }
  }
  if (active && l == 0) xyzz_store_g(D + ((u64)a * J.out_stride + J.out_off + idx - 1u) * XYZZ_WORDS, acc);
}
__global__ void __launch_bounds__(256) k_digit_final(const u32 *__restrict__ X, u32 *__restrict__ Eout, DigitJobs jobs, DigitJobs jtop, u32 top_w) {
  raise_priority(jobs.prio);
  __shared__ u32 s_val[16 * LDS_STRIDE];
  const u32 r = blockIdx.x & 3u, tid = threadIdx.x;
  const bool is_top = (blockIdx.x >> 2) >= top_w;
  const u32 a = is_top ? (blockIdx.x >> 2) - top_w : (blockIdx.x >> 2);
  const DigitJob J = is_top ? jtop.j[r] : jobs.j[r];
  const u32 idx = (tid >> 4) + 1u, l = tid & 15u;
  xyzz acc;
  xyzz_set_inf(acc);
  if (idx <= J.nsums) {
    const u32 *base = X + ((u64)a * J.in_stride + J.in_off) * XYZZ_WORDS;
    if (J.type == 0) {
      for (u32 hi = l; ((hi << J.s) | idx) <= J.N; hi += 16u) {
        xyzz x;
        xyzz_load_g(x, base + (u64)(((hi << J.s) | idx) - 1u) * XYZZ_WORDS);
        xyzz_add(acc, acc, x);
      }
    } else {
      for (u32 lo = l; lo < (1u << J.s) && ((idx << J.s) | lo) <= J.N; lo += 16u) {
        xyzz x;
        xyzz_load_g(x, base + (u64)(((idx << J.s) | lo) - 1u) * XYZZ_WORDS);
        xyzz_add(acc, acc, x);
      }
    }
  }
  for (u32 m = 1; m < 16u; m <<= 1) {
    xyzz other;
    xyzz_shfl_xor(other, acc, (int)m);
    xyzz_add(acc, acc, other);
  }
  if (l == 0) xyzz_store(s_val + (idx - 1u) * LDS_STRIDE, acc);
  __syncthreads();
  if (tid >= 64u) return;
  xyzz val;
  xyzz_set_inf(val);
  if (tid < J.nsums) xyzz_load(val, s_val + tid * LDS_STRIDE);
  for (u32 d = 1; d < 16; d <<= 1) {
    xyzz other;
    xyzz_shfl_down16(other, val, (int)d);
    if (l + d < 16u) xyzz_add(val, val, other);
  }
  for (u32 m = 1; m < 16; m <<= 1) {
    xyzz other;
    xyzz_shfl_xor(other, val, (int)m);
    xyzz_add(val, val, other);
  }
  if (tid == 0) xyzz_store_g(Eout + (u64)blockIdx.x * XYZZ_WORDS, val);
}

#define QP_SWAP2 0x4E
#define QP_B0 0x00
#define QP_B1 0x55
#define QP_B2 0xAA
#define QP_B3 0xFF
template <int CTRL> __device__ __forceinline__ void fe_quad(fe &r, const fe &s) {
#pragma unroll
  for (int k = 0; k < 9; k++) {
    u32 v = (u32)__builtin_amdgcn_update_dpp(0, (int)s.v[k], CTRL, 0xF, 0xF, false);
    asm volatile("" : "+v"(v));
    r.v[k] = v;
  }
}
template <int CTRL> __device__ __forceinline__ u32 u32_quad(u32 v) { return (u32)__builtin_amdgcn_update_dpp(0, (int)v, CTRL, 0xF, 0xF, false); }
__device__ __forceinline__ void fe_select(fe &r, bool c, const fe &x, const fe &y) {
#pragma unroll
  for (int k = 0; k < 9; k++) r.v[k] = c ? x.v[k] : y.v[k];
}
__device__ __forceinline__ void quad_add(fe &a, const fe &b, u32 q) {
  const bool lo = q < 2u;
  const u32 infA = u32_quad<QP_B2>(fe_is_zero_tight(a) ? 1u : 0u), infB = u32_quad<QP_B2>(fe_is_zero_tight(b) ? 1u : 0u);
  fe bx, r1, o1, t, u;
  fe_quad<QP_SWAP2>(bx, b);
  fe_mul(r1, a, bx);
  fe_quad<QP_SWAP2>(o1, r1);
  fe_select(u, lo, o1, r1);
  fe_select(t, lo, r1, o1);
  fe_sub(t, u, t);
  fe_carry(t, t);
  const u32 z = fe_is_zero_tight(t) ? 1u : 0u;
  const u32 pz = u32_quad<QP_B0>(z), rz = u32_quad<QP_B1>(z);
  fe opa, opb, r2, r3, r4, ppb, tmp;
  fe_select(opa, lo, t, a);
  fe_select(opb, lo, t, b);
  fe_mul(r2, opa, opb);
  fe_quad<QP_B0>(ppb, r2);
  fe_quad<QP_B0>(tmp, r1);
  fe_select(opa, q == 0u, t, r2);
  fe_select(opa, q == 1u, tmp, opa);
  fe_mul(r3, opa, ppb);
  fe pppb, x3, qx;
  fe_quad<QP_B0>(pppb, r3);
  fe_sub(x3, r2, pppb);
  fe_add(tmp, r3, r3);
  fe_sub_m2(x3, x3, tmp);
  fe_carry(x3, x3);
  fe_sub(qx, r3, x3);
  fe_quad<QP_B1>(tmp, r1);
  fe_select(opa, q == 0u, tmp, r2);
  fe_select(opa, q == 1u, t, opa);
  fe_select(opb, q == 1u, qx, pppb);
  fe_mul(r4, opa, opb);
  fe y3;
  fe_quad<QP_B0>(tmp, r4);
  fe_sub(y3, r4, tmp);
  fe_carry(y3, y3);
  fe x3b, res;
  fe_quad<QP_B1>(x3b, x3);
  fe_select(res, q == 0u, x3b, y3);
  fe_select(res, q == 2u, r3, res);
  fe_select(res, q == 3u, r4, res);
  const bool dbl = !infA && !infB && pz && rz;
  if (__ballot(dbl)) {
    xyzz A;
    fe_quad<QP_B0>(A.X, a); fe_quad<QP_B1>(A.Y, a); fe_quad<QP_B2>(A.ZZ, a); fe_quad<QP_B3>(A.ZZZ, a);
    if (dbl) {
      xyzz D;
      xyzz_dbl(D, A);
      fe_select(res, q == 0u, D.X, D.Y);
      fe_select(res, q == 2u, D.ZZ, res);
      fe_select(res, q == 3u, D.ZZZ, res);
    }
  }
  fe zero;
  fe_set_zero(zero);
  fe_select(res, pz && !rz, zero, res);
  fe_select(res, infB != 0u, a, res);
  fe_select(res, infA != 0u, b, res);
  a = res;
}

__global__ void __launch_bounds__(1024) k_digit_final_quad(const u32 *__restrict__ X, u32 *__restrict__ Eout, DigitJobs jobs, DigitJobs jtop, u32 top_w) {
  __shared__ u32 s_val[16 * XYZZ_WORDS];
  const u32 r = blockIdx.x & 3u, tid = threadIdx.x;
  const bool is_top = (blockIdx.x >> 2) >= top_w;
  const u32 a_idx = is_top ? (blockIdx.x >> 2) - top_w : (blockIdx.x >> 2);
  const DigitJob J = is_top ? jtop.j[r] : jobs.j[r];
  const u32 wave = tid >> 6, lane = tid & 63u, e = lane >> 2, q = lane & 3u;
  const u32 idx = wave + 1u;
  fe a;
  fe_set_zero(a);
  if (idx <= J.nsums) {
    const u32 *base = X + ((u64)a_idx * J.in_stride + J.in_off) * XYZZ_WORDS;
    u32 rec = 0;
    if (J.type == 0) { const u32 b = (e << J.s) | idx; if (b <= J.N) rec = b; }
    else { const u32 b = (idx << J.s) | e; if (e < (1u << J.s) && b <= J.N) rec = b; }
    if (rec) {
      const u32 *p = base + (u64)(rec - 1u) * XYZZ_WORDS + q * 9u;
#pragma unroll
      for (int k = 0; k < 9; k++) a.v[k] = p[k];
    }
  }
#pragma unroll 1
  for (u32 m = 4; m < 64u; m <<= 1) {
    fe b;
#pragma unroll
    for (int k = 0; k < 9; k++) b.v[k] = (u32)__shfl_xor((int)a.v[k], (int)m, 64);
    quad_add(a, b, q);
  }
  if (e == 0) {
#pragma unroll
    for (int k = 0; k < 9; k++) s_val[wave * XYZZ_WORDS + q * 9u + k] = a.v[k];
  }
  __syncthreads();
  if (wave) return;
  fe_set_zero(a);
  if (e < J.nsums) {
#pragma unroll
    for (int k = 0; k < 9; k++) a.v[k] = s_val[e * XYZZ_WORDS + q * 9u + k];
  }
#pragma unroll 1
  for (u32 d = 1; d < 16u; d <<= 1) {
    fe b;
#pragma unroll
    for (int k = 0; k < 9; k++) { const u32 v = (u32)__shfl_down((int)a.v[k], (int)(4u * d), 64); b.v[k] = (e + d < 16u) ? v : 0u; }
    quad_add(a, b, q);
  }
#pragma unroll 1
  for (u32 m = 4; m < 64u; m <<= 1) {
    fe b;
#pragma unroll
    for (int k = 0; k < 9; k++) b.v[k] = (u32)__shfl_xor((int)a.v[k], (int)m, 64);
    quad_add(a, b, q);
  }
  if (e == 0) {
#pragma unroll
    for (int k = 0; k < 9; k++) Eout[(u64)blockIdx.x * XYZZ_WORDS + q * 9u + k] = a.v[k];
  }
}

template <int MODE> __global__ void __launch_bounds__(256) k_digit_final_spread(const u32 *__restrict__ X, u32 *F, u32 *ticket, u32 *__restrict__ Eout, DigitJobs jobs,
                                                                               DigitJobs jtop, u32 top_w) {
  raise_priority(jobs.prio);
  const u32 gw = blockIdx.x * (blockDim.x >> 6) + (threadIdx.x >> 6);
  const u32 arr = MODE == 2 ? gw : gw >> 4, wave = MODE == 2 ? 0u : gw & 15u, r = arr & 3u;
  const bool is_top = (arr >> 2) >= top_w;
  const u32 a_idx = is_top ? (arr >> 2) - top_w : (arr >> 2);
  const DigitJob J = is_top ? jtop.j[r] : jobs.j[r];
  const u32 lane = threadIdx.x & 63u, e = lane >> 2, q = lane & 3u;
  const u32 idx = wave + 1u;
  fe a;
  if (MODE != 2 && idx <= J.nsums) {
    fe_set_zero(a);
    const u32 *base = X + ((u64)a_idx * J.in_stride + J.in_off) * XYZZ_WORDS;
    u32 rec = 0;
    if (J.type == 0) { const u32 b = (e << J.s) | idx; if (b <= J.N) rec = b; }
    else { const u32 b = (idx << J.s) | e; if (e < (1u << J.s) && b <= J.N) rec = b; }
    if (rec) {
      const u32 *p = base + (u64)(rec - 1u) * XYZZ_WORDS + q * 9u;
#pragma unroll
      for (int k = 0; k < 9; k++) a.v[k] = p[k];
    }
#pragma unroll 1
    for (u32 m = 4; m < 64u; m <<= 1) {
      fe b;
#pragma unroll
      for (int k = 0; k < 9; k++) b.v[k] = (u32)__shfl_xor((int)a.v[k], (int)m, 64);
      quad_add(a, b, q);
    }
    if (e == 0) {
#pragma unroll
      for (int k = 0; k < 9; k++) F[((u64)arr * 16u + wave) * XYZZ_WORDS + q * 9u + k] = a.v[k];
    }
  }
  if (MODE == 1) return;
  if (MODE == 0) {
    __threadfence();
    u32 t = 0;
    if (lane == 0) t = atomicAdd(ticket + arr, 1u);
    t = (u32)__shfl((int)t, 0, 64);
    if (t != 15u) return;
    __threadfence();
  }
  fe_set_zero(a);
  if (e < J.nsums) {
#pragma unroll
    for (int k = 0; k < 9; k++) a.v[k] = F[((u64)arr * 16u + e) * XYZZ_WORDS + q * 9u + k];
  }
#pragma unroll 1
  for (u32 d = 1; d < 16u; d <<= 1) {
    fe b;
#pragma unroll
    for (int k = 0; k < 9; k++) { const u32 v = (u32)__shfl_down((int)a.v[k], (int)(4u * d), 64); b.v[k] = (e + d < 16u) ? v : 0u; }
    quad_add(a, b, q);
  }
#pragma unroll 1
  for (u32 m = 4; m < 64u; m <<= 1) {
    fe b;
#pragma unroll
    for (int k = 0; k < 9; k++) b.v[k] = (u32)__shfl_xor((int)a.v[k], (int)m, 64);
    quad_add(a, b, q);
  }
  if (e == 0) {
#pragma unroll
    for (int k = 0; k < 9; k++) Eout[(u64)arr * XYZZ_WORDS + q * 9u + k] = a.v[k];
  }
  if (MODE == 0 && lane == 0) ticket[arr] = 0u;
}

__global__ void __launch_bounds__(256) k_debug_quad_add(const u32 *__restrict__ ra, const u32 *__restrict__ rb, u32 n, u32 *__restrict__ out) {
  const u32 t = blockIdx.x * blockDim.x + threadIdx.x;
  u32 i = t >> 2;
  const u32 q = t & 3u;
  const bool live = i < n;
  if (!live) i = n - 1u;
  fe a, b;
#pragma unroll
  for (int k = 0; k < 9; k++) { a.v[k] = ra[(u64)i * XYZZ_WORDS + q * 9u + k]; b.v[k] = rb[(u64)i * XYZZ_WORDS + q * 9u + k]; }
  quad_add(a, b, q);
  if (live) {
#pragma unroll
    for (int k = 0; k < 9; k++) out[(u64)i * XYZZ_WORDS + q * 9u + k] = a.v[k];
  }
}

__global__ void __launch_bounds__(256) k_window_weighted_small(MsmGeom g, const u32 *__restrict__ buckets, u32 *__restrict__ Eout) {
  raise_priority(g.prio & PRIO_FINISH);
  __shared__ u32 s_val[256 * LDS_STRIDE];
  const u32 tid = threadIdx.x, w = blockIdx.x;
  xyzz val;
  if (tid < g.B) xyzz_load_g(val, buckets + ((u64)w * g.B + tid) * XYZZ_WORDS);
  else xyzz_set_inf(val);
  for (u32 d = 1; d < g.B; d <<= 1) {
    xyzz_store(s_val + tid * LDS_STRIDE, val);
    __syncthreads();
    if (tid + d < g.B) {
      xyzz other;
      xyzz_load(other, s_val + (tid + d) * LDS_STRIDE);
      xyzz_add(val, val, other);
    }
    __syncthreads();
  }
  block_tree_sum(val, s_val);
  if (tid == 0) xyzz_store_g(Eout + (u64)w * XYZZ_WORDS, val);
}

__global__ void __launch_bounds__(1024) k_window_weighted_small_quad(MsmGeom g, const u32 *__restrict__ buckets, u32 *__restrict__ Eout) {
  __shared__ u32 s_val[256 * XYZZ_WORDS];
  const u32 tid = threadIdx.x, w = blockIdx.x, rec = tid >> 2, q = tid & 3u;
  fe a;
  fe_set_zero(a);
  if (rec < g.B) {
    const u32 *p = buckets + ((u64)w * g.B + rec) * XYZZ_WORDS + q * 9u;
#pragma unroll
    for (int k = 0; k < 9; k++) a.v[k] = p[k];
  }
  u32 *mine = s_val + rec * XYZZ_WORDS + q * 9u;
#pragma unroll 1
  for (u32 d = 1; d < g.B; d <<= 1) {
#pragma unroll
    for (int k = 0; k < 9; k++) mine[k] = a.v[k];
    __syncthreads();
    fe b;
#pragma unroll
    for (int k = 0; k < 9; k++) b.v[k] = (rec + d < g.B) ? mine[d * XYZZ_WORDS + k] : 0u;
    __syncthreads();
    quad_add(a, b, q);
  }
#pragma unroll 1
  for (u32 d = (blockDim.x >> 3); d > 0; d >>= 1) {
#pragma unroll
    for (int k = 0; k < 9; k++) mine[k] = a.v[k];
    __syncthreads();
    fe b;
#pragma unroll
    for (int k = 0; k < 9; k++) b.v[k] = (rec < d) ? mine[d * XYZZ_WORDS + k] : 0u;
    __syncthreads();
    quad_add(a, b, q);
  }
  if (rec == 0) {
#pragma unroll
    for (int k = 0; k < 9; k++) Eout[(u64)w * XYZZ_WORDS + q * 9u + k] = a.v[k];
  }
}

__device__ __forceinline__ void msm_small_block(const Segs &segs, const MsmGeom &g, u32 *__restrict__ out, u32 *s_val, u32 S) {
  const u32 w = blockIdx.x, tid = threadIdx.x;
  xyzz acc;
  xyzz_set_inf(acc);
  for (u32 i = blockIdx.y * blockDim.x + tid; i < g.n; i += S * blockDim.x) {
    u32 b = 0, sign = 0;
    for_each_digit(segs, g, i, [&](u32 ww, u32 bb, u32 sg) { if (ww == w) { b = bb; sign = sg; } });
    affine P;
    load_affine(P, seg_point(segs, i));
    if (b == 0 || affine_is_inf(P)) continue;
    jac q;
    q.X = P.x; q.Y = P.y; fe_set_one(q.Z);
    int top = 31 - __clz((int)b);
    for (int bit = top - 1; bit >= 0; bit--) {
      jac_dbl(q, q);
      if ((b >> bit) & 1u) jac_madd(q, P.x, P.y);
    }
    xyzz t;
    t.X = q.X;
    if (sign) { fe ny; fe_neg(ny, q.Y); fe_carry(t.Y, ny); } else t.Y = q.Y;
    fe_sqr(t.ZZ, q.Z);
    fe_mul(t.ZZZ, t.ZZ, q.Z);
    xyzz_add(acc, acc, t);
  }
  for (u32 m = 1; m < 64u; m <<= 1) {
    xyzz other;
    xyzz_shfl_xor(other, acc, (int)m);
    xyzz_add(acc, acc, other);
  }
  const u32 wave = tid >> 6, nwaves = blockDim.x >> 6;
  if ((tid & 63u) == 0) xyzz_store(s_val + wave * LDS_STRIDE, acc);
  __syncthreads();
  if (wave == 0) {
    if (tid < nwaves) xyzz_load(acc, s_val + tid * LDS_STRIDE); else xyzz_set_inf(acc);
    for (u32 m = 1; m < 4u; m <<= 1) {
      xyzz other;
      xyzz_shfl_xor(other, acc, (int)m);
      xyzz_add(acc, acc, other);
    }
    if (tid == 0) xyzz_store_g(out + ((u64)w * S + blockIdx.y) * XYZZ_WORDS, acc);
  }
}
__global__ void __launch_bounds__(256) k_msm_small(Segs segs, MsmGeom g, u32 *__restrict__ out) {
  __shared__ u32 s_val[4 * LDS_STRIDE];
  msm_small_block(segs, g, out, s_val, gridDim.y);
}
struct SmallPair { Segs segs[2]; MsmGeom g[2]; u32 *out[2]; u32 S[2]; };
__global__ void __launch_bounds__(256) k_msm_small_pair(SmallPair p) {
  __shared__ u32 s_val[4 * LDS_STRIDE];
  const u32 job = blockIdx.z;
  if (blockIdx.y >= p.S[job]) return;
  msm_small_block(p.segs[job], p.g[job], p.out[job], s_val, p.S[job]);
}
__global__ void __launch_bounds__(64) k_small_combine(const u32 *__restrict__ part, u32 S, u32 *__restrict__ E) {
  const u32 w = blockIdx.x, l = threadIdx.x;
  xyzz acc;
  if (l < S) xyzz_load_g(acc, part + ((u64)w * S + l) * XYZZ_WORDS); else xyzz_set_inf(acc);
  for (u32 m = 1; m < S; m <<= 1) {
    xyzz other;
    xyzz_shfl_xor(other, acc, (int)m);
    xyzz_add(acc, acc, other);
  }
  if (l == 0) xyzz_store_g(E + (u64)w * XYZZ_WORDS, acc);
}

struct CombinePair { const u32 *part[2]; u32 S[2]; u32 *E[2]; };
__global__ void __launch_bounds__(64) k_small_combine_pair(CombinePair c) {
  const u32 w = blockIdx.x, l = threadIdx.x, job = blockIdx.y, S = c.S[job];
  if (S <= 1) return;
  xyzz acc;
  if (l < S) xyzz_load_g(acc, c.part[job] + ((u64)w * S + l) * XYZZ_WORDS); else xyzz_set_inf(acc);
  for (u32 m = 1; m < S; m <<= 1) {
    xyzz other;
    xyzz_shfl_xor(other, acc, (int)m);
    xyzz_add(acc, acc, other);
  }
  if (l == 0) xyzz_store_g(c.E[job] + (u64)w * XYZZ_WORDS, acc);
}

#define MID_B 64
#define MID_THREADS 512
struct MidPair { Segs segs[2]; MsmGeom g[2]; u32 *E[2]; };
__global__ void __launch_bounds__(MID_THREADS) k_msm_mid(MidPair p) {
  __shared__ u32 s_cnt[MID_B + 2], s_off[MID_B + 2], s_cur[MID_B + 2], s_lane0[MID_B + 2];
  __shared__ unsigned short s_dig[MID_NMAX];
  __shared__ u32 s_ent[MID_NMAX];
  __shared__ u32 s_key[MID_THREADS];
  __shared__ u32 s_val[MID_THREADS * LDS_STRIDE];
  __shared__ u32 s_bkt[MID_B * XYZZ_WORDS];
  const u32 job = blockIdx.y, w = blockIdx.x, tid = threadIdx.x;
  const MsmGeom g = p.g[job];
  const u32 n = g.n;
  const u32 parts = gridDim.z, part = blockIdx.z;
  const u32 i0 = (u32)((u64)n * part / parts), i1 = (u32)((u64)n * (part + 1u) / parts);
  if (tid < MID_B + 2) s_cnt[tid] = 0;
  for (u32 i = tid; i < MID_B * XYZZ_WORDS; i += MID_THREADS) s_bkt[i] = 0;
  __syncthreads();
  for (u32 i = i0 + tid; i < i1; i += MID_THREADS) {
    sc v;
    const bool neg = load_digit_source(v, p.segs[job], i);
    {
      u64 cy = 0;
#pragma unroll
      for (int k = 0; k < 8; k++) {
        u32 kw = 0;
#pragma unroll
        for (int j = 0; j < 36; j++) { const int bit = 6 + 7 * j; if ((bit >> 5) == k) kw |= 1u << (bit & 31); }
        cy += (u64)v.v[k] + kw;
        v.v[k] = (u32)cy;
        cy >>= 32;
      }
    }
    const u32 pos = MID_C * w, wi = pos >> 5, sh = pos & 31u;
    u32 lo_w = 0, hi_w = 0;
#pragma unroll
    for (int k = 0; k < 8; k++) { if ((u32)k == wi) lo_w = v.v[k]; if ((u32)k == wi + 1u) hi_w = v.v[k]; }
    const u32 field = (u32)((((u64)hi_w << 32) | lo_w) >> sh) & ((1u << MID_C) - 1u);
    int d = (int)field - (w + 1u < g.W ? (int)MID_B : 0);
    const u32 b = (u32)(d < 0 ? -d : d);
    const u32 sign = (d < 0 ? 1u : 0u) ^ (neg ? 1u : 0u);
    s_dig[i - i0] = (unsigned short)(b | ((b ? sign : 0u) << 15));
    if (b) atomicAdd(&s_cnt[b], 1u);
  }
  __syncthreads();
  if (tid == 0) {
    u32 E = 0;
    for (u32 b = 1; b <= MID_B; b++) { s_off[b] = E; s_cur[b] = E; E += s_cnt[b]; }
    s_off[MID_B + 1] = E;
    const u32 q = (E + (MID_THREADS - MID_B) - 1) / (MID_THREADS - MID_B);
    u32 L = 0;
    for (u32 b = 1; b <= MID_B; b++) { s_lane0[b] = L; L += q ? (s_cnt[b] + q - 1) / q : 0u; }
    s_lane0[MID_B + 1] = L;
  }
  __syncthreads();
  for (u32 i = i0 + tid; i < i1; i += MID_THREADS) {
    const u32 d = s_dig[i - i0], b = d & 0x7FFFu;
    if (b) s_ent[atomicAdd(&s_cur[b], 1u)] = i | ((d >> 15) << 31);
  }
  __syncthreads();
  const u32 TL = s_lane0[MID_B + 1];
  u32 key = 0xFFFFFFFFu;
  xyzz acc;
  xyzz_set_inf(acc);
  if (tid < TL) {
    u32 lo = 1, hi = MID_B;
    while (lo < hi) { const u32 mid = (lo + hi + 1) >> 1; if (s_lane0[mid] <= tid) lo = mid; else hi = mid - 1; }
    const u32 b = lo;
    key = b;
    const u32 lanes = s_lane0[b + 1] - s_lane0[b], j = tid - s_lane0[b];
    const u32 beg = s_off[b], end = s_off[b + 1];
    u32 pos = beg + j;
    u32 w_next[16];
    u32 e_next = 0;
    if (pos < end) { e_next = s_ent[pos]; load_entry_point<false>(w_next, p.segs[job], e_next & 0x7FFFFFFFu); }
    while (pos < end) {
      const u32 e = e_next;
      affine P;
      affine_from_words(P, w_next);
      pos += lanes;
      if (pos < end) { e_next = s_ent[pos]; load_entry_point<false>(w_next, p.segs[job], e_next & 0x7FFFFFFFu); }
      xyzz_madd_signed(acc, P, (e >> 31) != 0);
    }
  }
  s_key[tid] = key;
  __syncthreads();
  for (u32 d = 1; d < MID_THREADS; d <<= 1) {
    const bool act = tid >= d && key != 0xFFFFFFFFu && s_key[tid - d] == key;
    if (!__syncthreads_or(act)) break;
    xyzz_store(s_val + tid * LDS_STRIDE, acc);
    __syncthreads();
    if (act) {
      xyzz other;
      xyzz_load(other, s_val + (tid - d) * LDS_STRIDE);
      xyzz_add(acc, other, acc);
    }
    __syncthreads();
  }
  if (key != 0xFFFFFFFFu && (tid + 1 == MID_THREADS || s_key[tid + 1] != key)) xyzz_store(s_bkt + (key - 1u) * XYZZ_WORDS, acc);
  __syncthreads();
  const bool live = tid < 4 * MID_B;
  const u32 rec = tid >> 2, q4 = tid & 3u;
  fe a;
  fe_set_zero(a);
  if (live) {
#pragma unroll
    for (int k = 0; k < 9; k++) a.v[k] = s_bkt[rec * XYZZ_WORDS + q4 * 9u + k];
  }
  u32 *mine = s_val + (live ? rec : 0u) * XYZZ_WORDS + q4 * 9u;
#pragma unroll 1
  for (u32 d = 1; d < MID_B; d <<= 1) {
    if (live) {
#pragma unroll
      for (int k = 0; k < 9; k++) mine[k] = a.v[k];
    }
    __syncthreads();
    fe b;
    fe_set_zero(b);
    if (live) {
#pragma unroll
      for (int k = 0; k < 9; k++) b.v[k] = (rec + d < MID_B) ? mine[d * XYZZ_WORDS + k] : 0u;
    }
    __syncthreads();
    if (live) quad_add(a, b, q4);
  }
#pragma unroll 1
  for (u32 d = MID_B >> 1; d > 0; d >>= 1) {
    if (live) {
#pragma unroll
      for (int k = 0; k < 9; k++) mine[k] = a.v[k];
    }
    __syncthreads();
    fe b;
    fe_set_zero(b);
    if (live) {
#pragma unroll
      for (int k = 0; k < 9; k++) b.v[k] = (rec < d) ? mine[d * XYZZ_WORDS + k] : 0u;
    }
    __syncthreads();
    if (live) quad_add(a, b, q4);
  }
  if (!live) return;
  if (rec == 0) {
#pragma unroll
    for (int k = 0; k < 9; k++) p.E[job][((u64)w * parts + part) * XYZZ_WORDS + q4 * 9u + k] = a.v[k];
  }
}

template <u32 THREADS, u32 NMAX>
__device__ __forceinline__ void msm_mid_block(const Segs &segs, const MsmGeom &g, const u32 w, const u32 parts, const u32 part, u32 *const &Eout) {
  __shared__ u32 s_cnt[MID_B + 2], s_off[MID_B + 2], s_cur[MID_B + 2], s_lane0[MID_B + 2];
  __shared__ unsigned short s_dig[NMAX];
  __shared__ u32 s_ent[NMAX];
  __shared__ u32 s_key[THREADS];
  __shared__ u32 s_val[THREADS * LDS_STRIDE];
  __shared__ u32 s_bkt[MID_B * XYZZ_WORDS];
  const u32 tid = threadIdx.x;
  const u32 n = g.n;
  const u32 i0 = (u32)((u64)n * part / parts), i1 = (u32)((u64)n * (part + 1u) / parts);
  if (tid < MID_B + 2) s_cnt[tid] = 0;
  for (u32 i = tid; i < MID_B * XYZZ_WORDS; i += THREADS) s_bkt[i] = 0;
  __syncthreads();
  for (u32 i = i0 + tid; i < i1; i += THREADS) {
    sc v;
    const bool neg = load_digit_source(v, segs, i);
    {
      u64 cy = 0;
#pragma unroll
      for (int k = 0; k < 8; k++) {
        u32 kw = 0;
#pragma unroll
        for (int j = 0; j < 36; j++) { const int bit = 6 + 7 * j; if ((bit >> 5) == k) kw |= 1u << (bit & 31); }
        cy += (u64)v.v[k] + kw;
        v.v[k] = (u32)cy;
        cy >>= 32;
      }
    }
    const u32 pos = MID_C * w, wi = pos >> 5, sh = pos & 31u;
    u32 lo_w = 0, hi_w = 0;
#pragma unroll
    for (int k = 0; k < 8; k++) { if ((u32)k == wi) lo_w = v.v[k]; if ((u32)k == wi + 1u) hi_w = v.v[k]; }
    const u32 field = (u32)((((u64)hi_w << 32) | lo_w) >> sh) & ((1u << MID_C) - 1u);
    int d = (int)field - (w + 1u < g.W ? (int)MID_B : 0);
    const u32 b = (u32)(d < 0 ? -d : d);
    const u32 sign = (d < 0 ? 1u : 0u) ^ (neg ? 1u : 0u);
    s_dig[i - i0] = (unsigned short)(b | ((b ? sign : 0u) << 15));
    if (b) atomicAdd(&s_cnt[b], 1u);
  }
  __syncthreads();
  if (tid == 0) {
    u32 E = 0;
    for (u32 b = 1; b <= MID_B; b++) { s_off[b] = E; s_cur[b] = E; E += s_cnt[b]; }
    s_off[MID_B + 1] = E;
    const u32 q = (E + (THREADS - MID_B) - 1) / (THREADS - MID_B);
    u32 L = 0;
    for (u32 b = 1; b <= MID_B; b++) { s_lane0[b] = L; L += q ? (s_cnt[b] + q - 1) / q : 0u; }
    s_lane0[MID_B + 1] = L;
  }
  __syncthreads();
  for (u32 i = i0 + tid; i < i1; i += THREADS) {
    const u32 d = s_dig[i - i0], b = d & 0x7FFFu;
    if (b) s_ent[atomicAdd(&s_cur[b], 1u)] = i | ((d >> 15) << 31);
  }
  __syncthreads();
  const u32 TL = s_lane0[MID_B + 1];
  u32 key = 0xFFFFFFFFu;
  xyzz acc;
  xyzz_set_inf(acc);
  if (tid < TL) {
    u32 lo = 1, hi = MID_B;
    while (lo < hi) { const u32 mid = (lo + hi + 1) >> 1; if (s_lane0[mid] <= tid) lo = mid; else hi = mid - 1; }
    const u32 b = lo;
    key = b;
    const u32 lanes = s_lane0[b + 1] - s_lane0[b], j = tid - s_lane0[b];
    const u32 beg = s_off[b], end = s_off[b + 1];
    u32 pos = beg + j;
    u32 w_next[16];
    u32 e_next = 0;
    if (pos < end) { e_next = s_ent[pos]; load_entry_point<false>(w_next, segs, e_next & 0x7FFFFFFFu); }
    while (pos < end) {
      const u32 e = e_next;
      affine P;
      affine_from_words(P, w_next);
      pos += lanes;
      if (pos < end) { e_next = s_ent[pos]; load_entry_point<false>(w_next, segs, e_next & 0x7FFFFFFFu); }
      xyzz_madd_signed(acc, P, (e >> 31) != 0);
    }
  }
  s_key[tid] = key;
  __syncthreads();
  for (u32 d = 1; d < THREADS; d <<= 1) {
    const bool act = tid >= d && key != 0xFFFFFFFFu && s_key[tid - d] == key;
    if (!__syncthreads_or(act)) break;
    xyzz_store(s_val + tid * LDS_STRIDE, acc);
    __syncthreads();
    if (act) {
      xyzz other;
      xyzz_load(other, s_val + (tid - d) * LDS_STRIDE);
      xyzz_add(acc, other, acc);
    }
    __syncthreads();
  }
  if (key != 0xFFFFFFFFu && (tid + 1 == THREADS || s_key[tid + 1] != key)) xyzz_store(s_bkt + (key - 1u) * XYZZ_WORDS, acc);
  __syncthreads();
  const bool live = tid < 4 * MID_B;
  const u32 rec = tid >> 2, q4 = tid & 3u;
  fe a;
  fe_set_zero(a);
  if (live) {
#pragma unroll
    for (int k = 0; k < 9; k++) a.v[k] = s_bkt[rec * XYZZ_WORDS + q4 * 9u + k];
  }
  u32 *mine = s_val + (live ? rec : 0u) * XYZZ_WORDS + q4 * 9u;
#pragma unroll 1
  for (u32 d = 1; d < MID_B; d <<= 1) {
    if (live) {
#pragma unroll
      for (int k = 0; k < 9; k++) mine[k] = a.v[k];
    }
    __syncthreads();
    fe b;
    fe_set_zero(b);
    if (live) {
#pragma unroll
      for (int k = 0; k < 9; k++) b.v[k] = (rec + d < MID_B) ? mine[d * XYZZ_WORDS + k] : 0u;
    }
    __syncthreads();
    if (live) quad_add(a, b, q4);
  }
#pragma unroll 1
  for (u32 d = MID_B >> 1; d > 0; d >>= 1) {
    if (live) {
#pragma unroll
      for (int k = 0; k < 9; k++) mine[k] = a.v[k];
    }
    __syncthreads();
    fe b;
    fe_set_zero(b);
    if (live) {
#pragma unroll
      for (int k = 0; k < 9; k++) b.v[k] = (rec < d) ? mine[d * XYZZ_WORDS + k] : 0u;
    }
    __syncthreads();
    if (live) quad_add(a, b, q4);
  }
  if (!live) return;
  if (rec == 0) {
#pragma unroll
    for (int k = 0; k < 9; k++) Eout[((u64)w * parts + part) * XYZZ_WORDS + q4 * 9u + k] = a.v[k];
  }
}

struct GroupMsm {
  const u32 *gens, *gsc;
  const u32 *v_pts, *v_sc;
  const u32 *p_pts, *p_sc;
  u32 nshared, m, per, group, P, W;
  u32 *E;
};
template <u32 THREADS, u32 NMAX> __global__ void __launch_bounds__(THREADS) k_msm_group(GroupMsm J) {
  const u32 t = blockIdx.x / J.W, w = blockIdx.x - t * J.W;
  const u32 g0 = t * J.group, cnt = min(J.group, J.P - g0);
  Segs s;
  s.pts[0] = J.gens; s.sc[0] = J.gsc + 8ull * J.nshared * t; s.n[0] = J.nshared;
  s.pts[1] = J.v_pts + 16ull * J.m * g0; s.sc[1] = J.v_sc + 8ull * J.m * g0; s.n[1] = cnt * J.m;
  s.pts[2] = J.p_pts + 16ull * J.per * g0; s.sc[2] = J.p_sc + 8ull * J.per * g0; s.n[2] = cnt * J.per;
  s.total = s.n[0] + s.n[1] + s.n[2];
  s.hlog[0] = s.hlog[1] = s.hlog[2] = 0xFFu;
  s.phase[0] = s.phase[1] = s.phase[2] = 0;
  s.glv_sub = nullptr; s.glv_neg = nullptr; s.glv_bx = nullptr;
  MsmGeom g = {};
  g.n = s.total; g.c = MID_C; g.W = J.W; g.B = MID_B;
  u32 *const Et = J.E + (u64)t * J.W * XYZZ_WORDS;
  msm_mid_block<THREADS, NMAX>(s, g, w, 1u, 0u, Et);
}
template __global__ void k_msm_group<MID_THREADS, MID_NMAX>(GroupMsm);
template __global__ void k_msm_group<GROUP_LIGHT_THREADS, GROUP_LIGHT_NMAX>(GroupMsm);

BPMI_HD void msm_tail_combine(u32 out_words[16], const u32 *E, u32 W, u32 c, const TailOffs &to) {
  const u32 o0 = to.off[0], o1 = to.nv > 1 ? to.off[1] : 0xFFFFFFFFu, o2 = to.nv > 2 ? to.off[2] : 0xFFFFFFFFu,
            o3 = to.nv > 3 ? to.off[3] : 0xFFFFFFFFu;
  xyzz acc;
  xyzz_set_inf(acc);
  u32 w = W, r = 0;
  for (u32 pos = W * c + to.top; pos-- > 0;) {
    if (r == 0) { w--; r = c + ((to.top && w + to.top >= W) ? 1u : 0u); }
    r--;
    xyzz_dbl(acc, acc);
    const bool tw = to.top && w + to.top >= W;
    const u32 v = tw ? (r == to.top_off[0] ? 0u : r == to.top_off[1] ? 1u : r == to.top_off[2] ? 2u : r == to.top_off[3] ? 3u : 4u)
                     : (r == o0 ? 0u : r == o1 ? 1u : r == o2 ? 2u : r == o3 ? 3u : 4u);
    if (v < 4u) {
      xyzz e;
      xyzz_load(e, E + ((u64)w * to.nv + v) * XYZZ_WORDS);
      xyzz_add(acc, acc, e);
    }
  }
  affine r_aff;
  xyzz_to_affine(r_aff, acc);
  affine_to_words(out_words, r_aff);
}
__global__ void __launch_bounds__(64) k_tail(const u32 *__restrict__ E, u32 W, u32 c, TailOffs to, u32 *__restrict__ out) {
  if (threadIdx.x == 0 && blockIdx.x == 0) {
    u32 w16[16];
    msm_tail_combine(w16, E, W, c, to);
#pragma unroll
    for (int i = 0; i < 16; i++) out[i] = w16[i];
  }
}

__global__ void __launch_bounds__(64) k_group_tail(const u32 *__restrict__ E, u32 W, u32 c, u32 ngroups, u32 *__restrict__ out) {
  const u32 t = blockIdx.x * 64u + threadIdx.x;
  if (t >= ngroups) return;
  TailOffs to;
  to.nv = 1; to.off[0] = to.off[1] = to.off[2] = to.off[3] = 0;
  u32 w16[16];
  msm_tail_combine(w16, E + (u64)t * W * XYZZ_WORDS, W, c, to);
  store_words16(out + 16ull * t, w16);
}

struct BatchMsm {
  const u32 *pts[3], *sc[3];
  u32 n[3];
  u32 W, parts, v0;
  u32 *E;
};
template <u32 THREADS, u32 NMAX> __global__ void __launch_bounds__(THREADS) k_msm_batch(BatchMsm J) {
  const u32 t = blockIdx.x / J.W, w = blockIdx.x - t * J.W;
  const u64 v = (u64)J.v0 + t;
  Segs s;
#pragma unroll
  for (int k = 0; k < 3; k++) { s.pts[k] = J.pts[k]; s.sc[k] = J.sc[k] + 8ull * J.n[k] * v; s.n[k] = J.n[k]; }
  s.total = s.n[0] + s.n[1] + s.n[2];
  s.hlog[0] = s.hlog[1] = s.hlog[2] = 0xFFu;
  s.phase[0] = s.phase[1] = s.phase[2] = 0;
  s.glv_sub = nullptr; s.glv_neg = nullptr; s.glv_bx = nullptr;
  MsmGeom g = {};
  g.n = s.total; g.c = MID_C; g.W = J.W; g.B = MID_B;
  u32 *const Et = J.E + (u64)t * J.W * J.parts * XYZZ_WORDS;
  msm_mid_block<THREADS, NMAX>(s, g, w, J.parts, blockIdx.z, Et);
}
template __global__ void k_msm_batch<MID_THREADS, MID_NMAX>(BatchMsm);
template __global__ void k_msm_batch<GROUP_LIGHT_THREADS, GROUP_LIGHT_NMAX>(BatchMsm);

__global__ void __launch_bounds__(64) k_msm_batch_tail(const u32 *__restrict__ E, u32 W, u32 c, u32 parts, u32 nvec, u32 *__restrict__ out) {
  const u32 t = blockIdx.x * 64u + threadIdx.x;
  if (t >= nvec) return;
  const u32 *Et = E + (u64)t * W * parts * XYZZ_WORDS;
  xyzz acc;
  xyzz_set_inf(acc);
#pragma unroll 1
  for (u32 w = W; w-- > 0;) {
#pragma unroll 1
    for (u32 r = 0; r < c; r++) xyzz_dbl(acc, acc);
#pragma unroll 1
    for (u32 p = 0; p < parts; p++) {
      xyzz e;
      xyzz_load(e, Et + ((u64)w * parts + p) * XYZZ_WORDS);
      xyzz_add(acc, acc, e);
    }
  }
  affine r_aff;
  xyzz_to_affine(r_aff, acc);
  u32 w16[16];
  affine_to_words(w16, r_aff);
  store_words16(out + 16ull * t, w16);
}

#if defined(BPMI_ISA_PROBE)
__global__ void __launch_bounds__(256) k_isa_probe_madd(u32 *__restrict__ accs, const u32 *__restrict__ xy) {
  const u32 t = blockIdx.x * blockDim.x + threadIdx.x;
  xyzz acc;
  xyzz_load(acc, accs + 36ull * t);
  fe x2, y2, P, R, nY;
#pragma unroll
  for (int k = 0; k < 9; k++) { x2.v[k] = xy[18ull * t + k]; y2.v[k] = xy[18ull * t + 9 + k]; }
  asm volatile("; BPMI_MARK madd_main_begin");
  xyzz_madd_pr(P, R, nY, acc, x2, y2);
  xyzz_madd_finish(acc, P, R, nY);
  asm volatile("; BPMI_MARK madd_main_end");
  xyzz_store(accs + 36ull * t, acc);
}
#endif
```

### python-bulletproofs_amd/csrc/msm_plan_host.hpp

```cpp
#pragma once
#include <algorithm>

#include "shared_defs.hpp"

struct MsmGeom {
  u32 n;
  u32 c;
  u32 W;
  u32 w0;
  u32 B;
  u32 G;
  u32 L;
  u32 nv;
  u32 prio;
  u32 fuse;
  u32 top2;
  u32 runs;
  u32 inblock;
};
struct DigitJob {
  u32 in_off, in_stride;
  u32 N, s, type;
  u32 glanes, gpw;
  u32 nsums;
  u32 out_off, out_stride;
  u32 blk0;
  u32 cnt;
};
struct DigitJobs { DigitJob j[4]; u32 njobs, prio; };

struct MsmMode {
  bool chained = false;
  bool free_run = false;
  bool beside = false;
};
struct MsmPlan { MsmGeom g; bool mid, small, glv; };
static inline bool msm_lds_sort(u32 c, u32 n) { return c >= 10u && n <= (1u << 23); }

#define MID_SINGLE_MAX_MIXED 5632u
static inline u32 pick_window_bits(const BpmiOptions &o, uint64_t n) {
  if (o.opt_c >= 2 && o.opt_c <= 16) return (u32)o.opt_c;
  if (o.opt_mixed && o.opt_top2) {
    if (n >= 185000u) return 16;
    if (n >= 19000u) return 13;
    if (n >= MID_SINGLE_MAX_MIXED) return 12;
  } else {
    if (n >= (1u << 17)) return 16;
    if (n >= 15360u) return o.opt_top2 ? 15 : 16;
    if (n >= 10240u) return 12;
  }
  if (n >= (1u << 10)) return 8;
  u32 lg = 0;
  while ((1ull << (lg + 1)) <= n) lg++;
  const int c = (int)lg - 2;
  return (u32)(c < 4 ? 4 : c);
}

#define SMALL_N_DEFAULT 4608
#define MID_MIN_DEFAULT 1536
#define MID_SINGLE_MIN_DEFAULT 2560

static inline u32 mid_parts(const BpmiOptions &o, uint64_t n) {
  if (o.opt_mid_parts >= 1 && o.opt_mid_parts <= 4) return (u32)o.opt_mid_parts;
  return n >= 3000u ? 3u : 1u;
}

static inline MsmPlan msm_pick_geometry(const BpmiOptions &o, const MsmMode &mode, uint64_t n, u32 w0, u32 wcount) {
  MsmPlan pl{};
  MsmGeom &g = pl.g;
  g.n = (u32)n;
  const uint64_t small_max = o.opt_small < 0 ? 0 : (o.opt_small ? (uint64_t)o.opt_small : SMALL_N_DEFAULT);
  const uint64_t mid_single = o.opt_mid_single > 0 ? (uint64_t)o.opt_mid_single : MID_SINGLE_MIN_DEFAULT;
  const uint64_t mid_single_max = (o.opt_mixed && o.opt_top2 && o.opt_mid_single == 0 && o.opt_mid_parts == 1) ? MID_SINGLE_MAX_MIXED - 1u : MID_NMAX;
  const bool mid = pl.mid = o.opt_mid_single >= 0 && n >= mid_single && n <= mid_single_max && o.opt_c == 0 && wcount == 0 && o.opt_glv <= 0;
  const bool small = pl.small = !mid && n <= small_max && o.opt_c == 0 && wcount == 0;
  const bool glv = pl.glv = o.opt_glv > 0 && !small && wcount == 0 && n >= 2 && 2 * n <= (1ull << 23);
  if (glv) g.n = (u32)(2 * n);
  g.c = mid ? MID_C : (small ? SMALL_C : pick_window_bits(o, n));
  g.top2 = 0;
  if (g.c >= 10u && g.c <= 15u && !glv && !wcount && !mid && !small && o.opt_top2 && (g.c == 15u || o.opt_mixed)) g.top2 = 256u - (256u / g.c) * g.c;
  g.W = wcount ? wcount : (glv ? 128u / g.c + 1u : (g.top2 ? 256u / g.c : 255u / g.c + 1u));
  g.w0 = w0;
  g.B = 1u << (g.c - 1);
  g.G = (g.W + g.top2) * g.B;
  g.inblock = (o.opt_inblock && (n <= (1u << 15) || ((g.c == 16u || g.top2) && n <= (1u << 17)))) ? 1u : 0u;
  const u32 rounds = o.opt_rounds > 0 ? (u32)o.opt_rounds : 3u;
  const u32 L_lanes = (u32)std::max<uint64_t>(20, ((uint64_t)g.W * g.n + 64ull * 3072 * rounds - 1) / (64ull * 3072 * rounds));
  u32 L_one = 64u;
  {
    const uint64_t e_max = (uint64_t)g.W * n;
    auto chunks_for = [&](uint64_t waves) { return (u32)((e_max * 1000 + 64 * waves * 1005 - 1) / (64 * waves * 1005)); };
    const u32 l3 = chunks_for(3072), l2 = chunks_for(2048), l1 = chunks_for(1024);
    L_one = l3 >= 20u ? l3 : (l2 >= 3u ? l2 : (l1 < 2u ? 2u : l1));
    if (L_one > 64u) L_one = 64u;
  }
  g.L = o.opt_chunk > 0 ? (u32)o.opt_chunk : ((n >= (1u << 19) && (mode.chained || mode.beside)) ? L_lanes : L_one);
  g.nv = (g.B <= 256u) ? 1u : 4u;
  g.prio = o.opt_prio == 1 ? 15u : (o.opt_prio > 1 ? (u32)(o.opt_prio & 15) : 0u);
  g.fuse = o.opt_fuse ? 1u : 0u;
  const bool lds_sort = !mid && !small && msm_lds_sort(g.c, g.n);
  g.runs = 0;
  if (lds_sort && !glv && g.G >= 2048u && (o.opt_accum_runs == 2 || (o.opt_accum_runs == 1 && g.c == 16u && !wcount && n >= (1u << 19)))) g.runs = 1;
  return pl;
}
static inline u32 msm_runs_cap(const BpmiOptions &o, const MsmGeom &g) {
  if (o.opt_accum_runs_cap > 0) return (u32)o.opt_accum_runs_cap;
  const uint64_t mean = ((uint64_t)g.n * g.W + g.G - 1) / g.G;
  return (u32)std::min<uint64_t>(2 * mean + 64, 1ull << 30);
}
static inline u32 msm_runs_bins(u32 cap) { return std::min<u32>(cap, RUN_BINS - 1u) + 1u; }
static inline u32 msm_runs_blocks(const MsmGeom &g) { return (g.G + RUN_SLICE - 1u) / RUN_SLICE; }

struct MsmWs {
  u32 *glv_sub, *glv_bx;
  unsigned char *glv_neg;
  u32 *dig, *hist, *off, *cursor, *bsum, *sidx, *buckets, *chunk_key, *coarse_hist, *coarse_off, *coarse_cursor;
  unsigned short *dig16;
  unsigned char *negs;
  u32 P;
  u32 *rec_key[2], *rec_pt[2];
  u32 *D, *E, *F, *out;
  u32 *run_order, *run_counts, *run_flags;
  size_t total;
  u32 nscan_blocks, rec0_max, nchunks;
};
static inline void msm_layout(const MsmGeom &g, MsmWs &w, char *base, bool glv = false) {
  size_t o = 0;
  auto take = [&](size_t bytes) { char *p = base ? base + o : nullptr; o += align_up(bytes, 256); return (u32 *)p; };
  w.glv_sub = take(glv ? 16ull * g.n : 0);
  w.glv_bx = take(glv ? 16ull * g.n : 0);
  w.glv_neg = (unsigned char *)take(glv ? g.n : 0);
  const size_t nW = (size_t)g.n * g.W;
  w.nscan_blocks = (u32)((g.G + SCAN_TILE - 1) / SCAN_TILE);
  w.nchunks = (u32)((nW + g.L - 1) / g.L);
  w.rec0_max = 2u * (g.fuse ? (w.nchunks + 63u) / 64u : w.nchunks);
  const u32 rec1_max = 2 * ((w.rec0_max + 255) / 256);
  w.P = msm_lds_sort(g.c, g.n) ? (g.G >> 8) : 0;
  w.hist = take(4ull * g.G);
  w.off = take(4ull * (g.G + 1));
  w.cursor = take(4ull * g.G);
  w.bsum = take(4ull * (w.nscan_blocks + 1));
  w.coarse_hist = take(4ull * COARSE_HIST_WORDS);
  w.coarse_off = take(4ull * (PART_MAX + 1));
  w.coarse_cursor = take(4ull * (PART_MAX + 1));
  w.dig = take(4ull * nW);
  w.sidx = take(4ull * nW);
  w.dig16 = (unsigned short *)take(w.P ? 2ull * nW : 0);
  w.negs = (unsigned char *)take(w.P ? g.n : 0);
  w.chunk_key = take(4ull * (w.nchunks + 1));
  w.buckets = take(4ull * XYZZ_WORDS * g.G);
  w.rec_key[0] = take(4ull * w.rec0_max);
  w.rec_pt[0] = take(4ull * XYZZ_WORDS * w.rec0_max);
  w.rec_key[1] = take(4ull * rec1_max);
  w.rec_pt[1] = take(4ull * XYZZ_WORDS * rec1_max);
  w.D = take(4ull * XYZZ_WORDS * g.W * (g.B > 256u ? (1u << ((g.c + 1u) / 2u)) + (1u << (g.c / 2u)) : 1u));
  w.E = take(4ull * XYZZ_WORDS * g.W * 4);
  w.F = take(4ull * XYZZ_WORDS * g.W * 64);
  w.out = take(64);
  w.run_order = w.cursor; w.run_counts = w.hist; w.run_flags = w.coarse_hist;
  w.total = o;
}

static inline u32 msb_index(u32 v) { u32 k = 0; while ((2u << k) <= v) k++; return k; }
static inline void digit_group(DigitJob &j, u32 elements, u32 epl) {
  u32 lanes = (elements + epl - 1u) / epl;
  if (lanes > 64u) lanes = 64u;
  if (lanes < 1u) lanes = 1u;
  j.gpw = 64u / lanes;
  j.glanes = 64u / j.gpw;
  if (j.glanes > elements) j.glanes = elements ? elements : 1u;
}
static inline u32 digit_job_waves(const DigitJobs &J, u32 k) {
  const uint64_t sums = (uint64_t)J.j[k].cnt * J.j[k].nsums;
  return (u32)((sums + J.j[k].gpw - 1u) / J.j[k].gpw);
}
static inline u32 digit_job_blocks(const DigitJobs &J, u32 k) { return (digit_job_waves(J, k) + 3u) / 4u; }
static inline DigitJobs digit_jobs2(u32 cnt, u32 in_off, u32 in_stride, u32 N, u32 s, u32 out_off, u32 out_stride, u32 epl) {
  DigitJobs J;
  memset(&J, 0, sizeof(J));
  J.njobs = 2;
  for (u32 type = 0; type < 2; type++) {
    DigitJob &j = J.j[type];
    j.cnt = cnt;
    j.in_off = in_off; j.in_stride = in_stride; j.N = N; j.s = s; j.type = type;
    j.nsums = type ? (N >> s) : ((1u << s) - 1u);
    digit_group(j, type ? (1u << s) : ((N - 1u) >> s) + 1u, epl);
    j.out_off = out_off + (type ? (1u << s) - 1u : 0u); j.out_stride = out_stride;
  }
  J.j[0].blk0 = 0;
  J.j[1].blk0 = digit_job_blocks(J, 0);
  return J;
}
static inline DigitJobs digit_jobs_concat(const DigitJobs &a, const DigitJobs &b) {
  DigitJobs J = a;
  u32 blk = a.j[1].blk0 + digit_job_blocks(a, 1);
  for (u32 k = 0; k < 2; k++) { J.j[2 + k] = b.j[k]; J.j[2 + k].blk0 = blk; blk += digit_job_blocks(b, k); }
  J.njobs = 4;
  return J;
}

struct MsmReducePlan {
  DigitJobs j1;
  DigitJobs j2, j2top;
  u32 grid1, top_w;
  TailOffs to;
};
static inline MsmReducePlan msm_reduce_plan(const MsmGeom &g, const BpmiOptions &o) {
  MsmReducePlan r{};
  r.to.nv = 1;
  r.top_w = 0xFFFFFFFFu;
  if (g.B <= 256u) return r;
  const u32 s0 = g.c / 2u, N0 = (1u << s0) - 1u, N1 = g.B >> s0;
  const u32 t0 = (s0 + 1u) / 2u, t1 = (msb_index(N1) + 1u) / 2u;
  const u32 stride1 = N0 + N1;
  const u32 Wr = g.W - g.top2;
  const u32 Bt = 2u * g.B, s0t = (g.c + 1u) / 2u, N0t = (1u << s0t) - 1u, N1t = Bt >> s0t;
  const u32 t0t = (s0t + 1u) / 2u, t1t = (msb_index(N1t) + 1u) / 2u;
  const u32 d_top = Wr * stride1, stride1t = N0t + N1t;
  auto stage1 = [&](u32 epl, DigitJobs &j) -> u32 {
    j = digit_jobs2(Wr, 0, g.B, g.B, s0, 0, stride1, epl);
    u32 waves = digit_job_waves(j, 0) + digit_job_waves(j, 1);
    if (g.top2) {
      DigitJobs jt = digit_jobs2(g.top2, Wr * g.B, Bt, Bt, s0t, d_top, stride1t, epl);
      waves += digit_job_waves(jt, 0) + digit_job_waves(jt, 1);
      j = digit_jobs_concat(j, jt);
    }
    return waves;
  };
  if (o.opt_epl > 0) stage1((u32)o.opt_epl, r.j1);
  else if (o.opt_reduce_fit) {
    u32 epl = 2;
    while (epl < 64u && stage1(epl, r.j1) > 1024u) epl++;
  } else {
    u32 epl = (u32)(((uint64_t)g.G) >> 15);
    stage1(epl < 2u ? 2u : (epl > 16u ? 16u : epl), r.j1);
  }
  r.j2 = digit_jobs_concat(digit_jobs2(Wr, 0, stride1, N0, t0, 0, 64, 1), digit_jobs2(Wr, N0, stride1, N1, t1, 0, 64, 1));
  r.to.nv = 4; r.to.off[0] = 0; r.to.off[1] = t0; r.to.off[2] = s0; r.to.off[3] = s0 + t1;
  if (g.top2) {
    r.j2top = digit_jobs_concat(digit_jobs2(g.top2, d_top, stride1t, N0t, t0t, 0, 64, 1), digit_jobs2(g.top2, d_top + N0t, stride1t, N1t, t1t, 0, 64, 1));
    r.to.top = g.top2; r.to.top_off[0] = 0; r.to.top_off[1] = t0t; r.to.top_off[2] = s0t; r.to.top_off[3] = s0t + t1t;
    r.top_w = Wr;
  }
  r.j1.prio = g.prio & PRIO_SUMS;
  r.j2.prio = r.j2top.prio = g.prio & PRIO_FINISH;
  r.grid1 = r.j1.j[r.j1.njobs - 1].blk0 + digit_job_blocks(r.j1, r.j1.njobs - 1);
  return r;
}

#define SLICE_N_DEFAULT (1u << 20)
#define SLICE_N_LIMIT (1u << 23)
static inline bool segs_dense(const Segs &s) { return s.hlog[0] >= 32u && s.hlog[1] >= 32u && s.hlog[2] >= 32u && !s.glv_sub; }
static inline Segs segs_slice(const Segs &s, uint64_t lo, uint64_t cnt) {
  Segs r = segs_init();
  u32 k = 0;
  uint64_t base = 0;
  for (int i = 0; i < 3; i++) {
    const uint64_t a = std::max<uint64_t>(lo, base), b = std::min<uint64_t>(lo + cnt, base + s.n[i]);
    if (b > a) { r.pts[k] = s.pts[i] + 16ull * (a - base); r.sc[k] = s.sc[i] + 8ull * (a - base); r.n[k] = (u32)(b - a); k++; }
    base += s.n[i];
  }
  r.total = (u32)cnt;
  return r;
}
struct MsmSlice { uint64_t lo, cnt; };
static inline MsmSlice msm_slice(uint64_t total, uint64_t per, uint64_t k) { return MsmSlice{k * per, std::min<uint64_t>(per, total - k * per)}; }
static inline uint64_t msm_slice_count(const BpmiOptions &o, const Segs &segs) {
  if (!segs_dense(segs) || o.opt_c || o.opt_split) return 1;
  const uint64_t slice_n = o.opt_slice_n < 0 ? SLICE_N_LIMIT : std::min<uint64_t>(o.opt_slice_n ? (uint64_t)o.opt_slice_n : SLICE_N_DEFAULT, SLICE_N_LIMIT);
  const uint64_t slice_min = o.opt_slice_n < 0 ? SLICE_N_LIMIT + 1 : (o.opt_slice_min ? (uint64_t)o.opt_slice_min : slice_n + slice_n / 2 + slice_n / 8);
  if (segs.total < slice_min && segs.total <= SLICE_N_LIMIT) return 1;
  const uint64_t cap = std::min<uint64_t>(slice_n + slice_n / 16, SLICE_N_LIMIT);
  return std::max<uint64_t>(2, (segs.total + cap - 1) / cap);
}
```

### python-bulletproofs_amd/csrc/shared_defs.hpp

```cpp
#pragma once
#include <stdint.h>
#include <string.h>

#include "../../include/bpmi.h"
#include "curve.hpp"

using bpmi::u32;
using bpmi::TailOffs;

#define XYZZ_WORDS 36
static inline size_t align_up(size_t x, size_t a) { return (x + a - 1) / a * a; }
static inline bool log2_exact(uint64_t n, u32 &k) { k = 0; while ((1ull << k) < n) k++; return n && (1ull << k) == n; }

struct Segs {
  const u32 *pts[3];
  const u32 *sc[3];
  u32 n[3];
  u32 total;
  u32 hlog[3];
  u32 phase[3];
  const u32 *glv_sub;
  const unsigned char *glv_neg;
  const u32 *glv_bx;
};
static inline Segs segs_init() {
  Segs s;
  memset(&s, 0, sizeof(s));
  s.hlog[0] = s.hlog[1] = s.hlog[2] = 0xFFu;
  return s;
}
static inline bool segs_one_dense(const Segs &s) {
  return s.total != 0 && s.n[0] == s.total && s.n[1] == 0 && s.n[2] == 0 && s.hlog[0] >= 32u && !s.glv_sub;
}

#define PRIO_SORT 1u
#define PRIO_SCAN 2u
#define PRIO_SUMS 4u
#define PRIO_FINISH 8u
#define PART_MAX 2048
#define COARSE_HIST_WORDS (PART_MAX + 192)
#define FINE_TILE 4096
#define RUN_FLAG_WORD (PART_MAX + 3)
#define RUN_COUNT_WORD (PART_MAX + 4)
#define RUN_BINS 1024u
#define RUN_SLICE 4096u
#define SCAN_PER_THREAD 16
#define SCAN_TILE (256 * SCAN_PER_THREAD)
#define SMALL_C 8
#define MID_C 7
#define MID_NMAX 8448
#define GROUP_LIGHT_THREADS 256
#define GROUP_LIGHT_NMAX 512

#define RP_ROLES 4
#define RP_MAX_PROOF_BYTES 32768u
#define CTX_SLOTS(k_, m_) (2u + 3u * (k_) + (m_))
#define RP_MIXED_MAX_CLASSES 64
#define RP_MIXED_UNIT_STRIDE 256
#define RP_UPLOAD_SLICES 4

struct BpmiOptions {
  int opt_c = 0;
  int opt_tail = 0;
  int opt_prio = 1;
  int opt_hist_threads = 0, opt_hist_blocks = 0;
  int opt_quad = 1;
  int opt_mulb = 1;
  int opt_chunk = 0;
  int opt_small = 0;
  int opt_fold_wnaf = 2;
  int opt_rp_only_role = -1;
  int opt_glv = 0;
  int opt_rp_prio = 1;
  int opt_rp_slices = 0;
  int opt_rp_overlap = 1;
  int opt_rp_rows = 0;
  int opt_rp_lanes = 0;
  int opt_epl = 0;
  int opt_tail_thread = 1;
  int opt_pair_chain = 0;
  int opt_mid_min = 0;
  int opt_mid_single = 0;
  int opt_pair1 = 1;
  int opt_fuse = 1;
  int opt_spin_wait = 0;
  int opt_async_lanes = 0;
  int opt_split = 0;
  int64_t opt_ipa_big = 0;
  int opt_ipa_step = 0;
  int opt_fold_shared = 1;
  int64_t opt_ipa_small = 0;
  int opt_ipa_fixed = 0;
  int opt_direct = 1;
  int opt_pair_phases = 0;
  int opt_graph = 0;
  int opt_mid_parts = 0;
  int opt_mixed = 1;
  int opt_top2 = 1;
  int opt_reduce_fit = 1;
  int opt_final_spread = 3;
  int opt_inblock = 1;
  int opt_prover_tw = 0;
  int opt_prover_job_lanes = 0;
  int opt_validate = 1;
  int opt_histscan = 0;
  int opt_segfuse = 0;
  int opt_slice_n = 0;
  int opt_slice_min = 0;
  int opt_pair_sched = 0;
  int opt_prover_wire = 2;
  int opt_prover_split = 0;
  int opt_rounds = 0;
  int opt_pair_rounds = 0;
  int opt_accum_chain = 1;
  int opt_accum_stream = 0;
  int opt_lane_prio = 0;
  int opt_accum_runs = 1;
  int opt_accum_runs_cap = 0;
  int opt_h2c_plain = 0;
  int opt_h2c_per_lane = 0;
  int opt_msm_batch_route = 0;
  int opt_msm_batch_vecs = 0;
};
```

Baseline: 1.253 billion pairs/s.

## Fold coarse scan, run counting and heavy scatter into fewer sort kernels

Measured after the change: 1.253 billion pairs/s (median of 2 runs). Within noise of the previous version (-0.0%).

```diff
diff --git a/python-bulletproofs_amd/csrc/msm_host.hpp b/python-bulletproofs_amd/csrc/msm_host.hpp
--- a/python-bulletproofs_amd/csrc/msm_host.hpp
+++ b/python-bulletproofs_amd/csrc/msm_host.hpp
@@ -91,37 +91,35 @@
   return BPMI_OK;
 }
 static void msm_queue_sort_lds(bpmi_ctx *ctx, hipStream_t st, const Segs &segs, const MsmGeom &g, const MsmWs &w, const MsmRecode *rec = nullptr) {
+  const u32 cap = g.runs ? msm_runs_cap(*ctx, g) : 0u, run_blocks = g.runs ? msm_runs_blocks(g) : 0u;
+  const RunTable rt = {w.run_order, w.run_counts, w.run_flags, g.runs ? msm_runs_bins(cap) : 0u, cap};
+  const bool counts_in_b = msm_runs_counted_by_level_b(g, rec != nullptr);
+  const RunTable rt_b = counts_in_b ? rt : RunTable{nullptr, nullptr, nullptr, 0u, 0u};
   {
     StageTimer t(ctx, ST_DIGITS, st);
     const u32 ht = ctx->opt_hist_threads > 0 ? (u32)ctx->opt_hist_threads : 1024u;
     const u32 hb = (u32)std::min<uint64_t>(((uint64_t)(rec ? rec->real.n : g.n) + ht - 1) / ht, ctx->opt_hist_blocks > 0 ? (u32)ctx->opt_hist_blocks : 256u);
-    CoarseScanOut so = {nullptr, nullptr, nullptr, nullptr};
-    if (ctx->opt_histscan && !rec) { so.coarse_off = w.coarse_off; so.coarse_cursor = w.coarse_cursor; so.offG = w.off + g.G; so.ticket = w.coarse_hist + PART_MAX + 2; }
     if (rec) hipLaunchKernelGGL(k_fixed_recode, dim3(hb), dim3(ht), 0, st, rec->sc, rec->real, rec->n_scalars, rec->R, rec->Wv, g, w.P, w.coarse_hist, w.dig16, w.negs);
-    else hipLaunchKernelGGL(k_coarse_hist, dim3(hb), dim3(ht), 0, st, segs, g, w.P, w.coarse_hist, w.dig16, w.negs, so);
+    else hipLaunchKernelGGL(k_coarse_hist, dim3(hb), dim3(ht), 0, st, segs, g, w.P, w.coarse_hist, w.dig16, w.negs, rt_b.counts, rt_b.nbins * run_blocks);
   }
   debug_sync(ctx, "ST_DIGITS", st);
-  if (!ctx->opt_histscan || rec) {
-    StageTimer t(ctx, ST_SCAN, st);
-    hipLaunchKernelGGL(k_coarse_scan, dim3(1), dim3(1024), 0, st, w.coarse_hist, w.P, w.coarse_off, w.coarse_cursor, w.off + g.G);
-  }
-  debug_sync(ctx, "ST_SCAN", st);
   {
     StageTimer t(ctx, ST_SCATTER, st);
     const u32 TS = g.n >= (1u << 19) ? PT_MAX : 4096u;
-    hipLaunchKernelGGL(k_partition, dim3((g.n + TS - 1) / TS, g.W), dim3(PT_THREADS), 0, st, g, w.P, TS, w.coarse_off, w.coarse_cursor, w.dig16, w.negs, w.dig,
+    hipLaunchKernelGGL(k_partition, dim3((g.n + TS - 1) / TS, g.W), dim3(PT_THREADS), 0, st, g, w.P, TS, w.coarse_hist, w.coarse_off, w.coarse_cursor, w.off + g.G, w.dig16, w.negs, w.dig,
                        w.hist, w.coarse_hist + PART_MAX);
-    const u32 nft = (u32)(((size_t)g.n * g.W + FINE_TILE - 1) / FINE_TILE);
+    const u32 heavy_blocks = msm_heavy_blocks(g);
     const u32 *any_heavy = w.coarse_hist + PART_MAX;
-    if (!g.inblock) hipLaunchKernelGGL(k_fine_hist_heavy, dim3(nft), dim3(256), 0, st, g, w.P, w.coarse_off, w.dig, w.coarse_off + w.P, any_heavy, w.hist);
-    hipLaunchKernelGGL(k_fine_sort_part, dim3(w.P), dim3(FINE_THREADS), 0, st, g, w.coarse_off, w.dig, w.hist, w.off, w.cursor, w.chunk_key, w.sidx, w.buckets);
-    if (!g.inblock) hipLaunchKernelGGL(k_fine_scatter_heavy, dim3(nft), dim3(256), 0, st, g, w.P, w.coarse_off, w.dig, w.coarse_off + w.P, any_heavy, w.cursor, w.sidx);
-    if (g.runs) {
-      const u32 cap = msm_runs_cap(*ctx, g), nblk = msm_runs_blocks(g);
-      const RunTable rt = {w.run_order, w.run_counts, w.run_flags, msm_runs_bins(cap), cap};
-      hipLaunchKernelGGL(k_runs_hist, dim3(nblk), dim3(256), 0, st, g, w.off, rt);
-      hipLaunchKernelGGL(k_runs_scatter, dim3(nblk), dim3(256), 0, st, g, w.off, rt);
-    }
+    if (heavy_blocks) hipLaunchKernelGGL(k_fine_hist_heavy, dim3(heavy_blocks), dim3(256), 0, st, g, w.P, w.coarse_off, w.dig, w.coarse_off + w.P, any_heavy, w.hist);
+    hipLaunchKernelGGL(k_fine_sort_part, dim3(w.P), dim3(FINE_THREADS), 0, st, g, w.coarse_off, w.dig, w.hist, w.off, w.cursor, w.chunk_key, w.sidx, w.buckets, rt_b, any_heavy);
+    if (g.runs && !counts_in_b) {
+      if (heavy_blocks) hipLaunchKernelGGL(k_fine_scatter_heavy, dim3(heavy_blocks), dim3(256), 0, st, g, w.P, w.coarse_off, w.dig, w.coarse_off + w.P, any_heavy, w.cursor, w.sidx);
+      hipLaunchKernelGGL(k_runs_hist, dim3(run_blocks), dim3(256), 0, st, g, w.off, rt);
+      hipLaunchKernelGGL(k_sort_tail, dim3(run_blocks), dim3(256), 0, st, g, w.P, run_blocks, w.off, rt, w.coarse_off, w.dig, w.coarse_off + w.P, any_heavy, w.cursor, w.sidx);
+    }
+    else if (!run_blocks && heavy_blocks) hipLaunchKernelGGL(k_fine_scatter_heavy, dim3(heavy_blocks), dim3(256), 0, st, g, w.P, w.coarse_off, w.dig, w.coarse_off + w.P, any_heavy, w.cursor, w.sidx);
+    else if (run_blocks) hipLaunchKernelGGL(k_sort_tail, dim3(run_blocks + heavy_blocks), dim3(256), 0, st, g, w.P, run_blocks, w.off, rt, w.coarse_off, w.dig,
+                                                      w.coarse_off + w.P, any_heavy, w.cursor, w.sidx);
   }
   debug_sync(ctx, "ST_SCATTER", st);
 }
@@ -149,7 +147,7 @@
 static int msm_queue_sort(bpmi_ctx *ctx, hipStream_t st, const Segs &segs, const MsmGeom &g, const MsmWs &w, const MsmRecode *rec = nullptr) {
   {
     StageTimer t(ctx, ST_MISC, st);
-    if (w.P) HIPCHK(ctx, hipMemsetAsync(w.coarse_hist, 0, 4ull * COARSE_HIST_WORDS, st));
+    if (w.P) HIPCHK(ctx, hipMemsetAsync(w.coarse_hist, 0, msm_sort_fill_bytes(), st));
     else {
       HIPCHK(ctx, hipMemsetAsync(w.hist, 0, 4ull * g.G, st));
       HIPCHK(ctx, hipMemsetAsync(w.buckets, 0, 4ull * XYZZ_WORDS * g.G, st));
diff --git a/python-bulletproofs_amd/csrc/msm_kernels.hpp b/python-bulletproofs_amd/csrc/msm_kernels.hpp
--- a/python-bulletproofs_amd/csrc/msm_kernels.hpp
+++ b/python-bulletproofs_amd/csrc/msm_kernels.hpp
@@ -103,12 +103,11 @@
 
 #define FINE_CAP 12288
 #define DIG_NONE 0xFFFFu
-struct CoarseScanOut { u32 *coarse_off, *coarse_cursor, *offG, *ticket; };
 __global__ void __launch_bounds__(1024) k_coarse_hist(Segs segs, MsmGeom g, u32 P, u32 *coarse_hist, unsigned short *__restrict__ dig16,
-                                                     unsigned char *__restrict__ negs, CoarseScanOut scan) {
+                                                     unsigned char *__restrict__ negs, u32 *__restrict__ run_counts, u32 run_words) {
   raise_priority(g.prio & PRIO_SORT);
   __shared__ u32 lh[PART_MAX];
-  __shared__ u32 s_last;
+  for (u32 i = blockIdx.x * blockDim.x + threadIdx.x; i < run_words; i += gridDim.x * blockDim.x) run_counts[i] = 0;
   for (u32 p = threadIdx.x; p < P; p += blockDim.x) lh[p] = 0;
   __syncthreads();
   const u32 Bc = g.B >> 8;
@@ -122,40 +121,8 @@
   }
   __syncthreads();
   for (u32 p = threadIdx.x; p < P; p += blockDim.x) { const u32 v = lh[p]; if (v) atomicAdd(&coarse_hist[p], v); }
-  if (!scan.ticket) return;
-  __threadfence();
-  __syncthreads();
-  if (threadIdx.x == 0) s_last = (atomicAdd(scan.ticket, 1u) == gridDim.x - 1u) ? 1u : 0u;
-  __syncthreads();
-  if (!s_last) return;
-  __threadfence();
-  const u32 tid = threadIdx.x, nt = blockDim.x, per = (P + nt - 1u) / nt;
-  u32 loc[8], sum = 0;
-#pragma unroll
-  for (u32 k = 0; k < 8u; k++) {
-    const u32 idx = tid * per + k;
-    loc[k] = (k < per && idx < P) ? __atomic_load_n(&coarse_hist[idx], __ATOMIC_RELAXED) : 0u;
-    sum += loc[k];
-  }
-  lh[tid] = sum;
-  __syncthreads();
-  for (u32 d = 1; d < nt; d <<= 1) {
-    const u32 v = tid >= d ? lh[tid - d] : 0u;
-    __syncthreads();
-    lh[tid] += v;
-    __syncthreads();
-  }
-  u32 excl = lh[tid] - sum;
-#pragma unroll
-  for (u32 k = 0; k < 8u; k++) {
-    const u32 idx = tid * per + k;
-    if (k < per && idx < P) { scan.coarse_off[idx] = excl; scan.coarse_cursor[idx] = excl; excl += loc[k]; }
-  }
-  if (tid == nt - 1u) { scan.coarse_off[P] = lh[tid]; *scan.offG = lh[tid]; }
-}
-__global__ void __launch_bounds__(1024) k_coarse_scan(const u32 *__restrict__ coarse_hist, u32 P, u32 *__restrict__ coarse_off,
-                                                      u32 *__restrict__ coarse_cursor, u32 *__restrict__ offG) {
-  __shared__ u32 sh[1024];
+}
+__device__ __forceinline__ void coarse_scan_block(const u32 *__restrict__ coarse_hist, u32 P, u32 *__restrict__ coarse_off, u32 *__restrict__ offG, u32 *sh) {
   const u32 tid = threadIdx.x;
   const u32 a = (2u * tid < P) ? coarse_hist[2u * tid] : 0u, b = (2u * tid + 1u < P) ? coarse_hist[2u * tid + 1u] : 0u;
   sh[tid] = a + b;
@@ -167,27 +134,28 @@
     __syncthreads();
   }
   const u32 excl = sh[tid] - (a + b);
-  if (2u * tid < P) { coarse_off[2u * tid] = excl; coarse_cursor[2u * tid] = excl; }
-  if (2u * tid + 1u < P) { coarse_off[2u * tid + 1u] = excl + a; coarse_cursor[2u * tid + 1u] = excl + a; }
+  if (2u * tid < P) coarse_off[2u * tid] = excl;
+  if (2u * tid + 1u < P) coarse_off[2u * tid + 1u] = excl + a;
   if (tid == 1023u) { coarse_off[P] = sh[1023]; *offG = sh[1023]; }
 }
 #define PT_MAX 16384
 #define PT_THREADS 1024u
 struct alignas(8) PartSigns { unsigned char b[8]; };
-__global__ void __launch_bounds__(PT_THREADS) k_partition(MsmGeom g, u32 P, u32 TS, const u32 *__restrict__ coarse_off, u32 *__restrict__ coarse_cursor,
-                                                          const unsigned short *__restrict__ dig16, const unsigned char *__restrict__ negs,
-                                                          u32 *__restrict__ part, u32 *__restrict__ fine_hist, u32 *__restrict__ any_heavy) {
+__global__ void __launch_bounds__(PT_THREADS) k_partition(MsmGeom g, u32 P, u32 TS, const u32 *__restrict__ coarse_hist, u32 *__restrict__ coarse_off,
+                                                          u32 *__restrict__ coarse_cursor, u32 *__restrict__ offG, const unsigned short *__restrict__ dig16,
+                                                          const unsigned char *__restrict__ negs, u32 *__restrict__ part, u32 *__restrict__ fine_hist,
+                                                          u32 *__restrict__ any_heavy) {
   constexpr u32 THREADS = PT_THREADS;
   static_assert((PT_MAX / 8u) % THREADS == 0u, "k_partition: whole vectors per thread");
   constexpr u32 NV = PT_MAX / 8u / THREADS;
   raise_priority(g.prio & PRIO_SORT);
-  __shared__ u32 cnt[128], excl[128], delta[128];
+  __shared__ u32 cnt[128], excl[128], delta[128], goff[128], s_red[THREADS / 64u];
   __shared__ u32 s_out[PT_MAX];
   const u32 w = blockIdx.y, tid = threadIdx.x;
   const u32 Bc0 = g.B >> 8, Bc = Bc0 << geom_wide(g, w), pbase = geom_slot(g, w) * Bc0;
   const u32 lin = blockIdx.y * gridDim.x + blockIdx.x, nblk = gridDim.x * gridDim.y;
   if (!g.inblock) for (u32 p = lin; p < P; p += nblk) {
-    if (coarse_off[p + 1] - coarse_off[p] > FINE_CAP) {
+    if (coarse_hist[p] > FINE_CAP) {
       if (tid < 256u) fine_hist[p * 256u + tid] = 0;
       if (tid == 0) *any_heavy = 1u;
     }
@@ -215,6 +183,14 @@
   }
   if (tid < nscal) { cs = dw[is]; ss = negs[is]; }
   if (tid < 128u) cnt[tid] = 0;
+  {
+    u32 front = 0;
+    for (u32 q = tid; q < pbase; q += THREADS) front += coarse_hist[q];
+#pragma unroll
+    for (u32 o = 32u; o; o >>= 1) front += (u32)__shfl_down((int)front, o, 64);
+    if ((tid & 63u) == 0u) s_red[tid >> 6] = front;
+  }
+  const u32 gc = (tid < 128u && tid < Bc) ? coarse_hist[pbase + tid] : 0u;
   __syncthreads();
 #pragma unroll
   for (u32 k = 0; k < NV; k++) {
@@ -228,20 +204,25 @@
   if (cs != DIG_NONE) atomicAdd(&cnt[(cs & 0x7FFFu) >> 8], 1u);
   __syncthreads();
   u32 c = 0;
-  if (tid < 128u) { c = tid < Bc ? cnt[tid] : 0u; excl[tid] = c; }
+  if (tid < 128u) { c = tid < Bc ? cnt[tid] : 0u; excl[tid] = c; goff[tid] = gc; }
   __syncthreads();
   for (u32 d = 1; d < 128u; d <<= 1) {
-    u32 v = 0;
-    if (tid < 128u && tid >= d) v = excl[tid - d];
-    __syncthreads();
-    if (tid < 128u) excl[tid] += v;
+    u32 v = 0, gv = 0;
+    if (tid < 128u && tid >= d) { v = excl[tid - d]; gv = goff[tid - d]; }
+    __syncthreads();
+    if (tid < 128u) { excl[tid] += v; goff[tid] += gv; }
     __syncthreads();
   }
   if (tid < 128u) {
     const u32 start = excl[tid] - c;
     excl[tid] = start;
     cnt[tid] = start;
-    if (c) delta[tid] = atomicAdd(&coarse_cursor[pbase + tid], c) - start;
+    if (c) {
+      u32 pstart = goff[tid] - gc;
+#pragma unroll
+      for (u32 k = 0; k < THREADS / 64u; k++) pstart += s_red[k];
+      delta[tid] = pstart + atomicAdd(&coarse_cursor[pbase + tid], c) - start;
+    }
   }
   __syncthreads();
 #pragma unroll
@@ -266,6 +247,10 @@
   for (u32 p = wave; p < Bc; p += nwaves) {
     const u32 lo = excl[p], hi = cnt[p], dl = delta[p];
     for (u32 j = lo + lane; j < hi; j += 64u) part[dl + j] = s_out[j];
+  }
+  if (lin == 0u) {
+    __syncthreads();
+    coarse_scan_block(coarse_hist, P, coarse_off, offG, s_out);
   }
 }
 #define CHUNK_FILL_OWN 16u
@@ -284,6 +269,7 @@
   }
 }
 #define FINE_THREADS 512
+struct RunTable { u32 *order, *counts, *flags; u32 nbins, cap; };
 __device__ __forceinline__ u32 lds_take_slot(u32 *bins, u32 bin) {
   const u32 lane = __builtin_amdgcn_mbcnt_hi(~0u, __builtin_amdgcn_mbcnt_lo(~0u, 0u));
   u32 pos = 0;
@@ -308,14 +294,19 @@
 }
 __global__ void __launch_bounds__(FINE_THREADS) k_fine_sort_part(MsmGeom g, const u32 *__restrict__ coarse_off, const u32 *__restrict__ part,
                                                                   const u32 *__restrict__ fine_hist, u32 *__restrict__ off, u32 *__restrict__ cursor,
-                                                                  u32 *__restrict__ chunk_key, u32 *__restrict__ sidx, u32 *__restrict__ buckets) {
+                                                                  u32 *__restrict__ chunk_key, u32 *__restrict__ sidx, u32 *__restrict__ buckets,
+                                                                  RunTable rt, const u32 *__restrict__ any_heavy) {
   raise_priority(g.prio & PRIO_SORT);
   __shared__ u32 bins[256];
   __shared__ u32 s_out[FINE_CAP];
+  static_assert(RUN_BINS <= FINE_CAP && RUN_SLICE % 256u == 0u, "k_fine_sort_part: the class counts borrow the staging buffer; whole partitions per slice");
   const u32 p = blockIdx.x, tid = threadIdx.x;
   const u32 base = coarse_off[p], m = coarse_off[p + 1] - base;
   const bool big = m > FINE_CAP;
   const bool heavy = big && !g.inblock;
+  const bool table = rt.nbins != 0u && !*any_heavy;
+  if (rt.nbins != 0u && !table && p == 0u && tid == 0u) rt.flags[RUN_FLAG_WORD] = 1u;
+  if (table) for (u32 i = tid; i < rt.nbins; i += FINE_THREADS) s_out[i] = 0;
   if (tid < 256u) bins[tid] = heavy ? fine_hist[p * 256u + tid] : 0u;
   __syncthreads();
   if (!heavy) {
@@ -342,10 +333,17 @@
       xyzz inf;
       xyzz_set_inf(inf);
       xyzz_store_g(buckets + (u64)key * XYZZ_WORDS, inf);
+    } else if (table) {
+      atomicAdd(&s_out[cnt < rt.nbins ? cnt : rt.nbins - 1u], 1u);
+      if (cnt > rt.cap) rt.flags[RUN_FLAG_WORD] = 1u;
     }
   }
   if (heavy) return;
   __syncthreads();
+  if (table) {
+    const u32 nblk = (g.G + RUN_SLICE - 1u) / RUN_SLICE, blk = p / (RUN_SLICE / 256u);
+    for (u32 i = tid; i < rt.nbins; i += FINE_THREADS) { const u32 v = s_out[i]; if (v) atomicAdd(&rt.counts[(rt.nbins - 1u - i) * nblk + blk], v); }
+  }
   if (tid < 256u) bins[tid] -= cnt;
   __syncthreads();
   if (big) {
@@ -367,11 +365,9 @@
   u32 j0, j1;
   u32 p_first;
 };
-__device__ __forceinline__ FineTile fine_tile_setup(const u32 *__restrict__ coarse_off, u32 P, u32 E, u32 *s_off) {
-  for (u32 i = threadIdx.x; i <= P; i += 256u) s_off[i] = coarse_off[i];
-  __syncthreads();
+__device__ __forceinline__ FineTile fine_tile_setup(u32 tile, u32 P, u32 E, const u32 *s_off) {
   FineTile t;
-  t.j0 = blockIdx.x * FINE_TILE;
+  t.j0 = tile * FINE_TILE;
   t.j1 = (t.j0 + FINE_TILE < E) ? t.j0 + FINE_TILE : E;
   u32 lo = 0, hi = P;
   while (hi - lo > 1) { const u32 mid = (lo + hi) >> 1; if (s_off[mid] <= t.j0) lo = mid; else hi = mid; }
@@ -390,59 +386,62 @@
   __shared__ u32 bins[FINE_BINS];
   if (!*any_heavy) return;
   const u32 E = offE[0];
-  if (blockIdx.x * FINE_TILE >= E) return;
-  const FineTile t = fine_tile_setup(coarse_off, P, E, s_off);
-  for (u32 i = threadIdx.x; i < FINE_BINS; i += 256u) bins[i] = 0;
-  __syncthreads();
-  const u32 g_first = t.p_first * 256u;
-  u32 pcur = t.p_first, bound = s_off[pcur + 1];
-  bool heavy = bound - s_off[pcur] > FINE_CAP;
-  for (u32 j = t.j0 + threadIdx.x; j < t.j1; j += 256u) {
-    if (j >= bound) { pcur = fine_partition_of(s_off, P, pcur, j); bound = s_off[pcur + 1]; heavy = bound - s_off[pcur] > FINE_CAP; }
-    if (heavy) {
-      const u32 key = pcur * 256u + (part[j] >> 24);
-      const u32 rel = key - g_first;
-      if (rel < FINE_BINS) atomicAdd(&bins[rel], 1u); else atomicAdd(&fine_hist[key], 1u);
-    }
-  }
-  __syncthreads();
-  for (u32 i = threadIdx.x; i < FINE_BINS; i += 256u) { const u32 v = bins[i]; if (v) atomicAdd(&fine_hist[g_first + i], v); }
-}
-__global__ void __launch_bounds__(256) k_fine_scatter_heavy(MsmGeom g, u32 P, const u32 *__restrict__ coarse_off, const u32 *__restrict__ part,
-                                                            const u32 *__restrict__ offE, const u32 *__restrict__ any_heavy, u32 *__restrict__ cursor,
-                                                            u32 *__restrict__ sidx) {
-  raise_priority(g.prio & PRIO_SORT);
-  __shared__ u32 s_off[PART_MAX + 1];
-  __shared__ u32 bins[FINE_BINS];
+  for (u32 i = threadIdx.x; i <= P; i += 256u) s_off[i] = coarse_off[i];
+  for (u32 tile = blockIdx.x; (u64)tile * FINE_TILE < E; tile += gridDim.x) {
+    __syncthreads();
+    const FineTile t = fine_tile_setup(tile, P, E, s_off);
+    for (u32 i = threadIdx.x; i < FINE_BINS; i += 256u) bins[i] = 0;
+    __syncthreads();
+    const u32 g_first = t.p_first * 256u;
+    u32 pcur = t.p_first, bound = s_off[pcur + 1];
+    bool heavy = bound - s_off[pcur] > FINE_CAP;
+    for (u32 j = t.j0 + threadIdx.x; j < t.j1; j += 256u) {
+      if (j >= bound) { pcur = fine_partition_of(s_off, P, pcur, j); bound = s_off[pcur + 1]; heavy = bound - s_off[pcur] > FINE_CAP; }
+      if (heavy) {
+        const u32 key = pcur * 256u + (part[j] >> 24);
+        const u32 rel = key - g_first;
+        if (rel < FINE_BINS) atomicAdd(&bins[rel], 1u); else atomicAdd(&fine_hist[key], 1u);
+      }
+    }
+    __syncthreads();
+    for (u32 i = threadIdx.x; i < FINE_BINS; i += 256u) { const u32 v = bins[i]; if (v) atomicAdd(&fine_hist[g_first + i], v); }
+  }
+}
+__device__ __forceinline__ void fine_scatter_heavy(u32 blk, u32 nblk, u32 P, const u32 *__restrict__ coarse_off, const u32 *__restrict__ part,
+                                                   const u32 *__restrict__ offE, const u32 *__restrict__ any_heavy, u32 *__restrict__ cursor,
+                                                   u32 *__restrict__ sidx, u32 *s_off, u32 *bins) {
   if (!*any_heavy) return;
   const u32 E = offE[0];
-  if (blockIdx.x * FINE_TILE >= E) return;
-  const FineTile t = fine_tile_setup(coarse_off, P, E, s_off);
-  for (u32 i = threadIdx.x; i < FINE_BINS; i += 256u) bins[i] = 0;
-  __syncthreads();
-  const u32 g_first = t.p_first * 256u;
-  u32 pcur = t.p_first, bound = s_off[pcur + 1];
-  bool heavy = bound - s_off[pcur] > FINE_CAP;
-  for (u32 j = t.j0 + threadIdx.x; j < t.j1; j += 256u) {
-    if (j >= bound) { pcur = fine_partition_of(s_off, P, pcur, j); bound = s_off[pcur + 1]; heavy = bound - s_off[pcur] > FINE_CAP; }
-    if (heavy) {
-      const u32 rel = pcur * 256u + (part[j] >> 24) - g_first;
-      if (rel < FINE_BINS) atomicAdd(&bins[rel], 1u);
-    }
-  }
-  __syncthreads();
-  for (u32 i = threadIdx.x; i < FINE_BINS; i += 256u) { const u32 v = bins[i]; if (v) bins[i] = atomicAdd(&cursor[g_first + i], v); }
-  __syncthreads();
-  pcur = t.p_first; bound = s_off[pcur + 1];
-  heavy = bound - s_off[pcur] > FINE_CAP;
-  for (u32 j = t.j0 + threadIdx.x; j < t.j1; j += 256u) {
-    if (j >= bound) { pcur = fine_partition_of(s_off, P, pcur, j); bound = s_off[pcur + 1]; heavy = bound - s_off[pcur] > FINE_CAP; }
-    if (heavy) {
-      const u32 e = part[j];
-      const u32 key = pcur * 256u + (e >> 24);
-      const u32 rel = key - g_first;
-      const u32 pos = (rel < FINE_BINS) ? atomicAdd(&bins[rel], 1u) : atomicAdd(&cursor[key], 1u);
-      sidx[pos] = (e & 0x7FFFFFu) | ((e & 0x800000u) << 8);
+  for (u32 i = threadIdx.x; i <= P; i += 256u) s_off[i] = coarse_off[i];
+  for (u32 tile = blk; (u64)tile * FINE_TILE < E; tile += nblk) {
+    __syncthreads();
+    const FineTile t = fine_tile_setup(tile, P, E, s_off);
+    for (u32 i = threadIdx.x; i < FINE_BINS; i += 256u) bins[i] = 0;
+    __syncthreads();
+    const u32 g_first = t.p_first * 256u;
+    u32 pcur = t.p_first, bound = s_off[pcur + 1];
+    bool heavy = bound - s_off[pcur] > FINE_CAP;
+    for (u32 j = t.j0 + threadIdx.x; j < t.j1; j += 256u) {
+      if (j >= bound) { pcur = fine_partition_of(s_off, P, pcur, j); bound = s_off[pcur + 1]; heavy = bound - s_off[pcur] > FINE_CAP; }
+      if (heavy) {
+        const u32 rel = pcur * 256u + (part[j] >> 24) - g_first;
+        if (rel < FINE_BINS) atomicAdd(&bins[rel], 1u);
+      }
+    }
+    __syncthreads();
+    for (u32 i = threadIdx.x; i < FINE_BINS; i += 256u) { const u32 v = bins[i]; if (v) bins[i] = atomicAdd(&cursor[g_first + i], v); }
+    __syncthreads();
+    pcur = t.p_first; bound = s_off[pcur + 1];
+    heavy = bound - s_off[pcur] > FINE_CAP;
+    for (u32 j = t.j0 + threadIdx.x; j < t.j1; j += 256u) {
+      if (j >= bound) { pcur = fine_partition_of(s_off, P, pcur, j); bound = s_off[pcur + 1]; heavy = bound - s_off[pcur] > FINE_CAP; }
+      if (heavy) {
+        const u32 e = part[j];
+        const u32 key = pcur * 256u + (e >> 24);
+        const u32 rel = key - g_first;
+        const u32 pos = (rel < FINE_BINS) ? atomicAdd(&bins[rel], 1u) : atomicAdd(&cursor[key], 1u);
+        sidx[pos] = (e & 0x7FFFFFu) | ((e & 0x800000u) << 8);
+      }
     }
   }
 }
@@ -738,7 +737,6 @@
   }
 }
 
-struct RunTable { u32 *order, *counts, *flags; u32 nbins, cap; };
 template <u32 N> __device__ __forceinline__ void run_lengths(u32 (&len)[N], const u32 *__restrict__ off, u32 k0, u32 stride, u32 k1) {
 #pragma unroll
   for (u32 k = 0; k < N; k++) { const u32 key = k0 + k * stride; len[k] = key < k1 ? off[key + 1] - off[key] : 0u; }
@@ -761,15 +759,15 @@
   for (u32 i = threadIdx.x; i < rt.nbins; i += 256u) rt.counts[(rt.nbins - 1u - i) * gridDim.x + blockIdx.x] = bins[i];
   if (longer) rt.flags[RUN_FLAG_WORD] = 1u;
 }
-__global__ void __launch_bounds__(256) k_runs_scatter(MsmGeom g, const u32 *__restrict__ off, RunTable rt) {
-  raise_priority(g.prio & PRIO_SORT);
-  __shared__ u32 s_base[RUN_BINS];
-  __shared__ u32 s_wave[4][RUN_BINS];
-  __shared__ u32 s_scan[256];
+#define RUNS_SCATTER_LDS (5u * RUN_BINS + 256u)
+__device__ __forceinline__ void runs_scatter(u32 blk, u32 nblk, const MsmGeom &g, const u32 *__restrict__ off, const RunTable &rt, u32 *smem) {
+  u32 *s_base = smem;
+  u32 (*s_wave)[RUN_BINS] = reinterpret_cast<u32 (*)[RUN_BINS]>(smem + RUN_BINS);
+  u32 *s_scan = smem + 5u * RUN_BINS;
   if (rt.flags[RUN_FLAG_WORD]) return;
-  const u32 tid = threadIdx.x, nblk = gridDim.x;
+  const u32 tid = threadIdx.x;
   const u32 wave = tid >> 6, lane = tid & 63u;
-  const u32 k0 = blockIdx.x * RUN_SLICE + wave * (RUN_SLICE / 4u);
+  const u32 k0 = blk * RUN_SLICE + wave * (RUN_SLICE / 4u);
   const u32 k1 = (k0 + RUN_SLICE / 4u < g.G) ? k0 + RUN_SLICE / 4u : g.G;
   u32 len[RUN_SLICE / 256u];
   run_lengths(len, off, k0 + lane, 64u, k1);
@@ -792,14 +790,14 @@
     __syncthreads();
   }
   {
-    u32 run = s_scan[tid] - sum, row = i0 / nblk, blk = i0 % nblk;
+    u32 run = s_scan[tid] - sum, row = i0 / nblk, b = i0 % nblk;
     for (u32 i = i0; i < i1; i++) {
-      if (blk == blockIdx.x) s_base[rt.nbins - 1u - row] = run;
+      if (b == blk) s_base[rt.nbins - 1u - row] = run;
       run += rt.counts[i];
-      if (++blk == nblk) { blk = 0; row++; }
-    }
-  }
-  if (blockIdx.x == 0 && tid == 255u) rt.flags[RUN_COUNT_WORD] = s_scan[255];
+      if (++b == nblk) { b = 0; row++; }
+    }
+  }
+  if (blk == 0 && tid == 255u) rt.flags[RUN_COUNT_WORD] = s_scan[255];
 #pragma unroll
   for (u32 k = 0; k < RUN_SLICE / 256u; k++)
     if (len[k]) atomicAdd(&s_wave[wave][len[k] < rt.nbins ? len[k] : rt.nbins - 1u], 1u);
@@ -812,6 +810,22 @@
 #pragma unroll
   for (u32 k = 0; k < RUN_SLICE / 256u; k++)
     if (len[k]) rt.order[atomicAdd(&s_wave[wave][len[k] < rt.nbins ? len[k] : rt.nbins - 1u], 1u)] = k0 + lane + k * 64u;
+}
+__global__ void __launch_bounds__(256) k_fine_scatter_heavy(MsmGeom g, u32 P, const u32 *__restrict__ coarse_off, const u32 *__restrict__ part,
+                                                            const u32 *__restrict__ offE, const u32 *__restrict__ any_heavy, u32 *__restrict__ cursor,
+                                                            u32 *__restrict__ sidx) {
+  raise_priority(g.prio & PRIO_SORT);
+  __shared__ u32 smem[PART_MAX + 1u + FINE_BINS];
+  fine_scatter_heavy(blockIdx.x, gridDim.x, P, coarse_off, part, offE, any_heavy, cursor, sidx, smem, smem + PART_MAX + 1u);
+}
+__global__ void __launch_bounds__(256) k_sort_tail(MsmGeom g, u32 P, u32 run_blocks, const u32 *__restrict__ off, RunTable rt, const u32 *__restrict__ coarse_off,
+                                                   const u32 *__restrict__ part, const u32 *__restrict__ offE, const u32 *__restrict__ any_heavy,
+                                                   u32 *__restrict__ cursor, u32 *__restrict__ sidx) {
+  raise_priority(g.prio & PRIO_SORT);
+  constexpr u32 HEAVY_LDS = PART_MAX + 1u + FINE_BINS;
+  __shared__ u32 smem[HEAVY_LDS > RUNS_SCATTER_LDS ? HEAVY_LDS : RUNS_SCATTER_LDS];
+  if (blockIdx.x < run_blocks) runs_scatter(blockIdx.x, run_blocks, g, off, rt, smem);
+  else fine_scatter_heavy(blockIdx.x - run_blocks, gridDim.x - run_blocks, P, coarse_off, part, offE, any_heavy, cursor, sidx, smem, smem + PART_MAX + 1u);
 }
 template <bool DENSE> __device__ __forceinline__ void runs_load_point(u32 w[16], const Segs &segs, u32 idx) {
   if (DENSE) load_words16(w, segs.pts[0] + 16ull * idx);
diff --git a/python-bulletproofs_amd/csrc/msm_plan_host.hpp b/python-bulletproofs_amd/csrc/msm_plan_host.hpp
--- a/python-bulletproofs_amd/csrc/msm_plan_host.hpp
+++ b/python-bulletproofs_amd/csrc/msm_plan_host.hpp
@@ -110,7 +110,18 @@
 }
 static inline u32 msm_runs_bins(u32 cap) { return std::min<u32>(cap, RUN_BINS - 1u) + 1u; }
 static inline u32 msm_runs_blocks(const MsmGeom &g) { return (g.G + RUN_SLICE - 1u) / RUN_SLICE; }
-
+static inline bool msm_runs_counted_by_level_b(const MsmGeom &g, bool fixed_base) { return g.runs != 0u && !fixed_base; }
+static inline u32 msm_heavy_blocks(const MsmGeom &g) {
+  if (g.inblock) return 0u;
+  return (u32)std::min<uint64_t>(((uint64_t)g.n * g.W + FINE_TILE - 1) / FINE_TILE, FINE_HEAVY_BLOCKS);
+}
+static inline u32 msm_sort_tail_launches(const MsmGeom &g, bool fixed_base) {
+  const u32 heavy = msm_heavy_blocks(g) ? 1u : 0u;
+  if (g.runs && !msm_runs_counted_by_level_b(g, fixed_base)) return 2u * heavy + 3u;
+  return heavy + 1u + ((g.runs || heavy) ? 1u : 0u);
+}
+
+static inline size_t msm_sort_fill_bytes() { return align_up(4ull * COARSE_HIST_WORDS, 256) + 2 * align_up(4ull * (PART_MAX + 1), 256); }
 struct MsmWs {
   u32 *glv_sub, *glv_bx;
   unsigned char *glv_neg;
diff --git a/python-bulletproofs_amd/csrc/shared_defs.hpp b/python-bulletproofs_amd/csrc/shared_defs.hpp
--- a/python-bulletproofs_amd/csrc/shared_defs.hpp
+++ b/python-bulletproofs_amd/csrc/shared_defs.hpp
@@ -40,6 +40,7 @@
 #define PART_MAX 2048
 #define COARSE_HIST_WORDS (PART_MAX + 192)
 #define FINE_TILE 4096
+#define FINE_HEAVY_BLOCKS 512u
 #define RUN_FLAG_WORD (PART_MAX + 3)
 #define RUN_COUNT_WORD (PART_MAX + 4)
 #define RUN_BINS 1024u
```
